# wonjune-kang/llm-speech-summarization

Hardware: AMD Instinct MI355X
Metric: generated tokens/s of end-to-end generate_audio_response steps (encode + prefill + 256-token greedy decode), HuBERT-large -> Llama-3.2-3B; audio-sec/s reported beside it, encoder stage alone and in the pipeline (higher is better)
Workload: dtype bf16

## Files before the change

### llm-speech-summarization_amd/csrc/api.hip

```cpp
#include <stdarg.h>
#include <stdlib.h>

#include <atomic>
#include <mutex>

#include "common.h"

static thread_local char g_err[512] = "";

void sl_set_error(const char* fmt, ...) {
  va_list ap;
  va_start(ap, fmt);
  vsnprintf(g_err, sizeof(g_err), fmt, ap);
  va_end(ap);
}

extern "C" const char* sl_last_error(void) { return g_err; }

extern "C" int sl_version(void) { return SL_ABI_VERSION; }

extern "C" int sl_kv_quantize_e4m3_host(const float* x, uint8_t* out, int64_t n) {
  SL_CHECK_ARG(x != nullptr && out != nullptr && n >= 0, "sl_kv_quantize_e4m3_host: bad arguments");
  for (int64_t i = 0; i < n; ++i) out[i] = (uint8_t)sl_q8_e4m3(x[i]);
  return 0;
}

extern "C" int sl_device_arch(char* buf, int n) {
  SL_CHECK_ARG(buf != nullptr && n > 0, "sl_device_arch: bad buffer");
  int dev = 0;
  SL_HIP(hipGetDevice(&dev));
  hipDeviceProp_t prop;
  SL_HIP(hipGetDeviceProperties(&prop, dev));
  snprintf(buf, (size_t)n, "%s", prop.gcnArchName);
  return 0;
}

static std::atomic<const SlEnv*> g_env{nullptr};
static std::mutex g_env_mu;

static int env_int(const char* name, int dflt) {
  const char* e = getenv(name);
  return (e && e[0]) ? atoi(e) : dflt;
}

static const SlEnv* env_load() {
  SlEnv& e = *new SlEnv();
  e.compact_pin = env_int("SL_COMPACT_PIN", 1);
  e.tape_fuse = env_int("SL_TAPE_FUSE", 1);
  e.attn_bwd_kf = env_int("SL_ATTN_BWD_KF", 0);
  e.decode_prefetch = env_int("SL_DECODE_PREFETCH", 0);
  e.attn_fwd_st = env_int("SL_ATTN_FWD_ST", 1);
  e.conv0_fold = env_int("SL_CONV0_FOLD", 1);
  e.enc_wt_ahead = env_int("SL_ENC_WT_AHEAD", 1);
  e.rms_bwd_lean = env_int("SL_RMSBWD_LEAN", 2);
  e.glds_ring = env_int("SL_GLDS_RING", 4);
  if (e.glds_ring != 3 && e.glds_ring != 4 && e.glds_ring != 104 && e.glds_ring != 204) e.glds_ring = 0;
  e.splitk_slots = env_int("SL_SPLITK_SLOTS", 0);
  e.glds_dmab = env_int("SL_GLDS_DMAB", 0);
  e.tt_ring = env_int("SL_TT_RING", 1);
  e.split_k256 = env_int("SL_SPLIT_K256", 1);
  e.ring_max_tiles = env_int("SL_GLDS_RING_MAX_TILES", 0);
  e.attn_bwd_both = env_int("SL_ATTN_BWD_BOTH", 1);
  e.wgrad_stream_min_tok = env_int("SL_WGRAD_STREAM_MIN_TOK", 0);
  e.tt_batched = env_int("SL_TT_BATCHED", 1);
  e.ln_colred_inkernel = env_int("SL_LN_COLRED_INKERNEL", 0);
  e.stream_min_m = env_int("SL_STREAM_MIN_M", 26);
  if (e.stream_min_m < 16) e.stream_min_m = 26;
  e.disable_t256 = getenv("SL_DISABLE_T256") != nullptr;
  e.t256_min_tiles = env_int("SL_T256_MIN_TILES", 512);
  e.t256_min_k = env_int("SL_T256_MIN_K", 1024);
  e.t256_phased = env_int("SL_T256_PHASED", 1);
  e.t256_by_rounds_pad = env_int("SL_T256_BY_ROUNDS_PAD", 1);
  e.decode_tiled = env_int("SL_DECODE_TILED", 1);
  e.stream_k = env_int("SL_STREAM_K", 1);
  e.split_k = env_int("SL_SPLIT_K", 1);
  e.wgrad_tr = env_int("SL_WGRAD_TR", 1);
  e.tt_max_splits = env_int("SL_TT_MAX_SPLITS", 8);
  e.lnbwd_nw = env_int("SL_LNBWD_NW", 16);
  e.skinny_alt = env_int("SL_SKINNY_ALT", 0);
  e.prefill_share_prefix = env_int("SL_PREFILL_SHARE_PREFIX", 1);
  e.prefill_prune_last = env_int("SL_PREFILL_PRUNE_LAST", 1);
  e.gemm_ko = env_int("SL_GEMM_KO", 0);
  { const char* sp = getenv("SL_GEMM_STAMP_PTR"); e.gemm_stamp_ptr = (sp && sp[0]) ? strtoull(sp, nullptr, 16) : 0ull; }
  const char* g = getenv("SL_DISABLE_GLDS");
  e.disable_glds = (g && g[0] == '1') ? 1 : ((g && g[0] == '2') ? 2 : 0);
  e.direct_epilogue = env_int("SL_DIRECT_EPILOGUE", 0);
  e.gemm_gm = env_int("SL_GEMM_GM", 8);
  e.attn_full_min = env_int("SL_ATTN_FULL_MIN", 32);
  e.attn_force_split = getenv("SL_ATTN_FORCE_SPLIT") != nullptr;
  { const int ks = env_int("SL_ATTN_DECODE_KS", 128); e.attn_decode_ks = (ks == 64 || ks == 65) ? ks : 128; }
  e.attn_split_merge = env_int("SL_ATTN_SPLIT_MERGE", -1);
  e.attn_generic = env_int("SL_ATTN_GENERIC", 0);
  e.attn_qt = env_int("SL_ATTN_QT", 0);
  e.norm_single_row = env_int("SL_NORM_SINGLE_ROW", 0);
  e.no_ln_fold = env_int("SL_NO_LN_FOLD", 0);
  e.no_swap_epilogue = env_int("SL_NO_SWAP_EPILOGUE", 0);
  e.gemm_log = env_int("SL_GEMM_LOG", 0);
  e.no_wgrad_stream = env_int("SL_NO_WGRAD_STREAM", 0);
  e.stream_splits = e.stream_nwv = e.stream_mt = 0;
  e.stream_nl = env_int("SL_STREAM_NL", 0);
  e.stream_wide = env_int("SL_STREAM_WIDE", 1);
  e.stream_wsplits = env_int("SL_STREAM_WSPLITS", 0);
  e.stream_fixup = env_int("SL_STREAM_FIXUP", 0);
  const char* sc = getenv("SL_STREAM_CFG");
  if (sc && sc[0]) {
    int sp = 0, nwv = 0, mt = 0;
    const int n = sscanf(sc, "%d,%d,%d", &sp, &nwv, &mt);
    if (n >= 2) {
      if (sp >= 1 && sp <= 64) e.stream_splits = sp;
      if (nwv == 2 || nwv == 4) e.stream_nwv = nwv;
    }
    if (n == 3 && (mt == 8 || mt == 16)) e.stream_mt = mt;
  }
  return &e;
}

const SlEnv& sl_env() {
  const SlEnv* e = g_env.load(std::memory_order_acquire);
  if (!e) {
    std::lock_guard<std::mutex> lk(g_env_mu);
    e = g_env.load(std::memory_order_relaxed);
    if (!e) {
      e = env_load();
      g_env.store(e, std::memory_order_release);
    }
  }
  return *e;
}

static thread_local int g_family_rows = 0;
int sl_family_rows(int rows) { return g_family_rows > rows ? g_family_rows : rows; }
int sl_family_pin(int rows) {
  const int prev = g_family_rows;
  g_family_rows = rows > 0 ? rows : 0;
  return prev;
}

extern "C" int sl_tuning_reload(void) {
  std::lock_guard<std::mutex> lk(g_env_mu);
  g_env.store(env_load(), std::memory_order_release);
  return 0;
}
```

### llm-speech-summarization_amd/csrc/common.h

```cpp
#pragma once
#include <hip/hip_runtime.h>
#include <stdint.h>
#include <stdio.h>
#include <string.h>

#include "../../include/speechllm.h"

void sl_set_error(const char* fmt, ...);

#define SL_CHECK_ARG(cond, ...)      \
  do {                               \
    if (!(cond)) {                   \
      sl_set_error(__VA_ARGS__);     \
      return SL_ERR_ARG;             \
    }                                \
  } while (0)

#define SL_CHECK_LAUNCH(what)                                                        \
  do {                                                                               \
    hipError_t e__ = hipGetLastError();                                              \
    if (e__ != hipSuccess) {                                                         \
      sl_set_error("%s: %s", what, hipGetErrorString(e__));                          \
      return SL_ERR_LAUNCH;                                                          \
    }                                                                                \
// ... 196 lines not shown
  }
};

__device__ __forceinline__ float gelu_erf(float x) { return 0.5f * x * (1.0f + erff(x * 0.70710678118654752440f)); }
__device__ __forceinline__ float gelu_fast(float x) {
  const float z = fabsf(x) * 0.70710678118654752440f;
  const float t = __builtin_amdgcn_rcpf(__builtin_fmaf(0.3275911f, z, 1.0f));
  float pl = __builtin_fmaf(0.5f * 1.061405429f, t, 0.5f * -1.453152027f);
  pl = __builtin_fmaf(pl, t, 0.5f * 1.421413741f);
  pl = __builtin_fmaf(pl, t, 0.5f * -0.284496736f);
  pl = __builtin_fmaf(pl, t, 0.5f * 0.254829592f);
  const float w = pl * t * __builtin_amdgcn_exp2f(-1.4426950408889634f * z * z);
  return __builtin_fmaf(-fabsf(x), w, fmaxf(x, 0.f));
}
__device__ __forceinline__ uint32_t lowbias32(uint32_t x) {
  x ^= x >> 16; x *= 0x7feb352du; x ^= x >> 15; x *= 0x846ca68bu; x ^= x >> 16;
  return x;
}
__device__ __forceinline__ bool dropout_keep(int64_t i, uint64_t seed, uint32_t thr24) {
  const uint32_t h = lowbias32((uint32_t)i ^ lowbias32((uint32_t)((uint64_t)i >> 32) ^ (uint32_t)seed) ^ (uint32_t)(seed >> 32));
  return (h >> 8) >= thr24;
}
__device__ __forceinline__ uint32_t drop_inner(uint32_t hi, uint64_t seed) { return lowbias32(hi ^ (uint32_t)seed) ^ (uint32_t)(seed >> 32); }
__device__ __forceinline__ bool dropout_keep_lo(uint32_t lo, uint32_t inner, uint32_t thr24) { return (lowbias32(lo ^ inner) >> 8) >= thr24; }
template <typename T> __device__ __forceinline__ float gelu_act(float x) {
  if constexpr (sizeof(T) == 2) return gelu_fast(x);
  else return gelu_erf(x);
}
__device__ __forceinline__ float silu(float x) { return x / (1.0f + __expf(-x)); }
__device__ __forceinline__ float gelu_grad(float u) {
  const float cdf = 0.5f * (1.0f + erff(u * 0.70710678118654752440f));
  const float pdf = 0.39894228040143267794f * __expf(-0.5f * u * u);
  return cdf + u * pdf;
}

__device__ __forceinline__ float wave_sum(float v) {
#pragma unroll
  for (int o = 32; o > 0; o >>= 1) v += __shfl_xor(v, o, 64);
  return v;
}
__device__ __forceinline__ float wave_max(float v) {
#pragma unroll
  for (int o = 32; o > 0; o >>= 1) v = fmaxf(v, __shfl_xor(v, o, 64));
  return v;
}

constexpr int SL_MAX_DEVICES = 64;

static inline int64_t ceil_div64(int64_t a, int64_t b) { return (a + b - 1) / b; }

#define SL_DISPATCH_DTYPE_INF(dtype, T, ...)                  \
  do {                                                        \
    if ((dtype) == SL_F32) {                                  \
      using T = float;                                        \
      __VA_ARGS__;                                            \
    } else if ((dtype) == SL_BF16) {                          \
      using T = bf16_t;                                       \
      __VA_ARGS__;                                            \
    } else if ((dtype) == SL_F16) {                           \
      using T = f16_t;                                        \
      __VA_ARGS__;                                            \
    } else {                                                  \
      sl_set_error("unknown dtype %d", (int)(dtype));         \
      return SL_ERR_ARG;                                      \
    }                                                         \
  } while (0)
#define SL_DISPATCH_DTYPE(dtype, T, ...)                      \
  do {                                                        \
    if ((dtype) == SL_F32) {                                  \
      using T = float;                                        \
      __VA_ARGS__;                                            \
    } else if ((dtype) == SL_BF16) {                          \
      using T = bf16_t;                                       \
      __VA_ARGS__;                                            \
    } else {                                                  \
      sl_set_error("unknown dtype %d", (int)(dtype));         \
      return SL_ERR_ARG;                                      \
    }                                                         \
  } while (0)

static inline size_t sl_dtype_size(int dtype) { return dtype == SL_F32 ? 4 : 2; }
static inline bool sl_is16(int dtype) { return dtype == SL_BF16 || dtype == SL_F16; }
static inline int sl_kv_format_check(const char* who, int kv_format, int dtype, int head_dim) {
  if (kv_format != SL_KV_MODEL_DTYPE && kv_format != SL_KV_FP8_E4M3) {
    sl_set_error("%s: unknown K/V cache format %d (0 = model dtype, 1 = fp8 e4m3)", who, kv_format);
    return SL_ERR_ARG;
  }
  if (kv_format == SL_KV_FP8_E4M3 && !sl_is16(dtype)) {
    sl_set_error("%s: the fp8 K/V cache is built for bf16 / fp16 models, not dtype %d (float32 is the parity mode)", who, dtype);
    return SL_ERR_UNSUPPORTED;
  }
  if (kv_format == SL_KV_FP8_E4M3 && head_dim != 128) {
    sl_set_error("%s: the fp8 K/V cache is built for head_dim 128, not %d", who, head_dim);
    return SL_ERR_UNSUPPORTED;
  }
  return 0;
}
static inline size_t sl_kv_elem_size(int kv_format, int dtype) { return kv_format == SL_KV_FP8_E4M3 ? 1 : sl_dtype_size(dtype); }

struct SlEnv {
  int attn_fwd_st;
  int conv0_fold;
  int enc_wt_ahead;
  int glds_ring;
  int tt_batched;
  int wgrad_stream_min_tok;
  int attn_bwd_both;
  int ring_max_tiles;
  int split_k256;
  int ln_colred_inkernel;
  int tt_ring;
  int glds_dmab;
  int splitk_slots;
  int rms_bwd_lean;
  int decode_prefetch;
  int attn_bwd_kf;
  int tape_fuse;
  int compact_pin;
  int stream_min_m;
  int disable_t256;
  int t256_min_tiles;
  int t256_min_k;
  int t256_by_rounds_pad;
  int t256_phased;
  int disable_glds;
  int direct_epilogue;
  int gemm_gm;
  int attn_full_min;
  int attn_force_split;
  int attn_decode_ks;
  int attn_split_merge;
  int attn_generic;
  int attn_qt;
  int norm_single_row;
  int no_ln_fold;
  int no_wgrad_stream;
  int gemm_log;
  int no_swap_epilogue;
  int decode_tiled;
  int prefill_share_prefix;
  int prefill_prune_last;
  int skinny_alt;
  int tt_max_splits;
  int lnbwd_nw;
  int wgrad_tr;
  int split_k;
  int stream_k;
  int gemm_ko;
  unsigned long long gemm_stamp_ptr;
  int stream_splits, stream_nwv, stream_mt;
  int stream_wide;
  int stream_wsplits;
  int stream_fixup;
  int stream_nl;
};
const SlEnv& sl_env();

#define SL_TRANSPOSE_BATCH 64
struct SlTransposeRec {
  const void* x; void* y;
  int64_t ldx, ldy;
  int32_t rows, cols, ld_out, tiles_r;
};
struct SlTransposeBatch {
  SlTransposeRec rec[SL_TRANSPOSE_BATCH];
  int32_t first_block[SL_TRANSPOSE_BATCH];
  int32_t n, pad;
};
int sl_transpose_pad_batch_impl(const SlTransposeRec* recs, int n, int32_t dtype, sl_stream stream);
int sl_family_rows(int rows);
int sl_family_pin(int rows);
struct SlFamilyPin {
  int prev;
  explicit SlFamilyPin(int rows) : prev(sl_family_pin(rows)) {}
  ~SlFamilyPin() { sl_family_pin(prev); }
};
```

### llm-speech-summarization_amd/csrc/gemm.hip

```cpp
#include <stdlib.h>

#include "common.h"
#include "gemm_internal.h"

#include "gemm_epilogue.h"

template <typename T, int ACT>
__global__ __launch_bounds__(256, 2) void gemm_tiled_kernel(GemmP p) {
  constexpr int VEC = Vec16<T>::VEC;
  constexpr int BK = TROWB / (int)sizeof(T);
  __shared__ __attribute__((aligned(16))) unsigned char smem[2][2][TBM * TROWB];

  const int tid = threadIdx.x, lane = tid & 63, wave = tid >> 6;
  const int wm = wave >> 1, wn = wave & 1;
  const int r = lane & 15, q = lane >> 4;

  int bm, bn;
  tile_patch_coords(xcd_remap(blockIdx.x, p.tiles_m * p.tiles_n), p.tiles_m, p.tiles_n, 8, bm, bn);
  const int z = blockIdx.y;

  int64_t a_off; int wz;
  if (!resolve_group(p, z, bm, a_off, wz)) return;
  const T* A = (const T*)p.A + a_off;
  const T* W = (const T*)p.W + (int64_t)wz * p.sW + p.wx;
// ... 788 lines not shown
        if (p.post == SL_POST_DROPOUT) post_ok = !p.colsum && !p.ln_mr && !p.stats_out && (act == SL_ACT_GELU ? (p.aux && !p.res) : (p.res && !p.aux));
        if (p.post == SL_POST_GELU_BWD || p.post == SL_POST_SILU_MUL_BWD)
          post_ok = act == SL_ACT_NONE && !(p.post_ld & 7) && !((uintptr_t)p.post_in & 15) && (p.post == SL_POST_GELU_BWD || !p.colsum);
        if (swap_store_ok(p, e, true) && form && !p.grp && !p.amax_val && post_ok && (phased || (!p.post && !p.colsum))) {
          pl.form = phased ? SL_T256_PHASED_SW : SL_T256_PLAIN_SW;
#ifdef SL_GEMM_DEBUG
          if (act == SL_ACT_NONE && phased && !p.ln_mr && (e.gemm_stamp_ptr || e.gemm_ko))
            pl.form = SL_T256_DBG + (e.gemm_stamp_ptr ? 8 : (e.gemm_ko >= 1 && e.gemm_ko <= 4 ? e.gemm_ko : 6));
#endif
        }
      }
      return pl;
    }
  }
  pl.tile(p, TBM);
  pl.grid = dim3(pl.tiles_m * pl.tiles_n, batch);
  const bool glds = whole_slabs(p, bk) && (!p.grp_ext || p.grp_kslab) && glds_on(e);
  if ((p.post || p.colsum) && !glds) { pl.fam = TP_UNSUPPORTED; return pl; }
  if (es == 2 && ring_ok(p, batch, bk, e, cus)) { pl.fam = TP_RING128; pl.form = e.glds_ring; }
  else if (whole_slabs(p, bk) && !p.grp_ext && e.disable_glds == 2) { pl.fam = TP_GLDS128; pl.form = GLDS_PLAIN; }
  else if (glds) { pl.fam = TP_GLDS128; pl.form = (es == 2 && e.glds_dmab && !p.grp_ext) ? GLDS_DMAB : GLDS_ASM; }
  else pl.fam = TP_REG128;
  return pl;
}

static void log_plan(const TiledPlan& pl) {
  static const char* const fam[] = {"reg128", "glds128", "ring128", "t256", "sk", "tt", "unsupported"};
  static const char* const glds[] = {"asm", "dmab", "plain"}, * const t256[] = {"phased", "phased_sw", "plain", "plain_sw", "sk", "sk_sw"};
  static const char* const tt[] = {"two_stage", "ring", "batched"}, * const close[] = {"none", "reduce", "defer"};
  char num[16];
  snprintf(num, sizeof(num), pl.fam == TP_T256 ? "dbg%d" : "%d", pl.form);
  const bool k256 = (pl.fam == TP_T256 || pl.fam == TP_SK) && pl.form < 6;
  const char* form = pl.fam == TP_GLDS128 ? glds[pl.form] : k256 ? t256[pl.form] : pl.fam == TP_TT ? tt[pl.form] : (pl.fam == TP_RING128 || pl.fam == TP_T256) ? num : "none";
  fprintf(stderr, "SLPLAN fam=%s form=%s tm=%d tn=%d grid=%u,%u,%u S=%d krun=%d close=%s\n", fam[pl.fam], form, pl.tiles_m, pl.tiles_n, pl.grid.x, pl.grid.y,
          pl.grid.z, pl.S, pl.krun, close[pl.close]);
}

template <typename T, int ACT>
static int run_tiled(const GemmP& p0, const TiledPlan& pl, void* sk_ws, const SlEnv& e, hipStream_t st) {
  if (pl.fam == TP_UNSUPPORTED) {
    sl_set_error("sl_gemm_ex: post_op / colsum_out need whole 128-byte K slabs (K %% %d == 0) and the LDS-DMA kernels (SL_DISABLE_GLDS unset)", TROWB / (int)sizeof(T));
    return SL_ERR_UNSUPPORTED;
  }
  float* part = (float*)((unsigned char*)sk_ws + SK_FLAG_BYTES);
  GemmP p = pl.runs ? partial_gemm(p0, pl.runs, pl.S, pl.krun, part) : p0;
  p.tiles_m = pl.tiles_m; p.tiles_n = pl.tiles_n;
#ifdef SL_GEMM_DEBUG
  if (pl.fam == TP_T256 && pl.form >= SL_T256_DBG) p.stamp = (uint32_t*)(uintptr_t)e.gemm_stamp_ptr;
#endif
  if (pl.fam == TP_TT) SL_TRY(sl_gemm_tt_kernel_launch(p, pl.form, pl.grid, pl.krun, st));
  else if (pl.fam == TP_T256 || pl.fam == TP_SK)
    SL_TRY((sl_gemm256_launch<T, ACT>(p, pl.form, pl.grid, pl.fam == TP_SK ? sk_ws : nullptr, st)));
  else if (pl.fam == TP_RING128) SL_TRY((sl_gemm128_ring_launch<T, ACT>(p, pl.form, pl.grid, st)));
  else {
    if (pl.fam == TP_REG128) hipLaunchKernelGGL((gemm_tiled_kernel<T, ACT>), pl.grid, dim3(256), 0, st, p);
    else if (pl.form == GLDS_PLAIN) hipLaunchKernelGGL((gemm_tiled_glds_kernel<T, ACT, false>), pl.grid, dim3(256), 0, st, p);
    else if (pl.form == GLDS_ASM) hipLaunchKernelGGL((gemm_tiled_glds_kernel<T, ACT, true>), pl.grid, dim3(256), 0, st, p);
    else if constexpr (sizeof(T) == 2) hipLaunchKernelGGL((gemm_tiled_glds_kernel<T, ACT, true, true>), pl.grid, dim3(256), 0, st, p);
    SL_CHECK_LAUNCH("gemm_tiled");
  }
  if (pl.close == CLOSE_DEFER) *p0.defer = pl.S;
  if (pl.close == CLOSE_REDUCE) {
    const int64_t vecs = ((int64_t)p0.M * p0.N + 3) / 4;
    hipLaunchKernelGGL((splitk_reduce_kernel<T>), dim3((unsigned)((vecs + 255) / 256)), dim3(256), 0, st, part, pl.S, (int64_t)p0.M * p0.N, p0);
    SL_CHECK_LAUNCH("splitk_reduce");
  }
  return 0;
}

template <typename T, int MT, int ACT, int RF, int NW, int U, bool PACKED, bool KCONT = false, bool W8 = false>
static int launch_skinny_cfg(GemmP& p, const SkinnyX& sx, int batch, hipStream_t st) {
  dim3 grid((p.N + 16 * RF - 1) / (16 * RF), batch);
  hipLaunchKernelGGL((gemm_skinny_kernel<T, MT, ACT, RF, NW, U, PACKED, KCONT, W8>), grid, dim3(NW * 64), 0, st, p, sx);
  SL_CHECK_LAUNCH("gemm_skinny");
  return 0;
}

template <typename T, int MT, int ACT, bool PACKED>
static int launch_skinny_mt(GemmP& p, const SkinnyX& sx, int batch, const SlEnv& e, hipStream_t st) {
  constexpr bool PAIRS = (ACT == SL_ACT_SILU_MUL || ACT == SL_ACT_ROPE_KV);
  const int nfrag = (p.N + 15) / 16 * batch;
  if constexpr (MT == 1) {
    if constexpr (PACKED && sizeof(T) == 2 && !PAIRS) {
      if (nfrag < 256 && sl_family_rows(p.M) <= 8 && !(e.skinny_alt & 1)) {
        const int per_wave = p.K / 32 / 16;
        if (per_wave % 3 == 0) return launch_skinny_cfg<T, MT, ACT, 1, 16, 3, PACKED>(p, sx, batch, st);
        return launch_skinny_cfg<T, MT, ACT, 1, 16, 4, PACKED>(p, sx, batch, st);
      }
    }
    if (nfrag >= 1024) return launch_skinny_cfg<T, MT, ACT, 4, 4, 4, PACKED>(p, sx, batch, st);
    if (nfrag >= 256 || PAIRS) return launch_skinny_cfg<T, MT, ACT, 2, 8, 4, PACKED>(p, sx, batch, st);
    if constexpr (!PAIRS) return launch_skinny_cfg<T, MT, ACT, 1, 16, 2, PACKED>(p, sx, batch, st);
  } else if constexpr (MT == 2) {
    if (nfrag >= 1024) return launch_skinny_cfg<T, MT, ACT, 2, 8, 4, PACKED>(p, sx, batch, st);
    if (nfrag >= 256 || PAIRS) return launch_skinny_cfg<T, MT, ACT, 2, 16, 2, PACKED>(p, sx, batch, st);
    if constexpr (!PAIRS) return launch_skinny_cfg<T, MT, ACT, 1, 16, 2, PACKED>(p, sx, batch, st);
  } else {
    if (nfrag >= 1024) return launch_skinny_cfg<T, MT, ACT, 4, 8, 2, PACKED>(p, sx, batch, st);
    if (nfrag >= 256 || PAIRS) return launch_skinny_cfg<T, MT, ACT, 2, 16, 2, PACKED>(p, sx, batch, st);
    if constexpr (!PAIRS) return launch_skinny_cfg<T, MT, ACT, 1, 16, 2, PACKED>(p, sx, batch, st);
  }
  return 0;
}

template <typename T, int MT, int ACT, int RF, int NW, int UA = 4>
static int launch_skinny_w8_u(GemmP& p, const SkinnyX& sx, hipStream_t st) {
  const int pw = p.K / 64 / NW;
  if (pw % UA != 0 && pw % 3 == 0) return launch_skinny_cfg<T, MT, ACT, RF, NW, 3, true, false, true>(p, sx, 1, st);
  return launch_skinny_cfg<T, MT, ACT, RF, NW, UA, true, false, true>(p, sx, 1, st);
}
template <typename T, int MT, int ACT>
static int launch_skinny_w8_mt(GemmP& p, const SkinnyX& sx, hipStream_t st) {
  constexpr bool PAIRS = (ACT == SL_ACT_SILU_MUL || ACT == SL_ACT_ROPE_KV);
  const int nfrag = (p.N + 15) / 16;
  if (nfrag >= 1024) return launch_skinny_w8_u<T, MT, ACT, MT == 1 ? 4 : 2, MT == 1 ? 4 : 8>(p, sx, st);
  if (nfrag >= 256 || PAIRS) return launch_skinny_w8_u<T, MT, ACT, 2, MT == 1 ? 8 : 16, MT == 1 ? 4 : 2>(p, sx, st);
  if constexpr (!PAIRS) return launch_skinny_w8_u<T, MT, ACT, 1, 16>(p, sx, st);
  return 0;
}
template <typename T>
static int launch_skinny_w8(GemmP& p, const SkinnyX& sx, int act, hipStream_t st) {
  const bool mt1 = sl_family_rows(p.M) <= 16;
  switch (act) {
    case SL_ACT_NONE: return mt1 ? launch_skinny_w8_mt<T, 1, SL_ACT_NONE>(p, sx, st) : launch_skinny_w8_mt<T, 2, SL_ACT_NONE>(p, sx, st);
    case SL_ACT_SILU_MUL: return mt1 ? launch_skinny_w8_mt<T, 1, SL_ACT_SILU_MUL>(p, sx, st) : launch_skinny_w8_mt<T, 2, SL_ACT_SILU_MUL>(p, sx, st);
    default: return mt1 ? launch_skinny_w8_mt<T, 1, SL_ACT_ROPE_KV>(p, sx, st) : launch_skinny_w8_mt<T, 2, SL_ACT_ROPE_KV>(p, sx, st);
  }
}

template <typename T, int ACT>
static int launch_skinny(GemmP& p, const SkinnyX& sx, int batch, bool packed, const SlEnv& e, hipStream_t st) {
  if (packed) {
    if constexpr (ACT == SL_ACT_GELU) {
      sl_set_error("sl_gemm: packed weights are not built with the GELU epilogue");
      return SL_ERR_UNSUPPORTED;
    } else {
      if (sl_family_rows(p.M) <= 16) return launch_skinny_mt<T, 1, ACT, true>(p, sx, batch, e, st);
      if (sl_family_rows(p.M) <= 32) return launch_skinny_mt<T, 2, ACT, true>(p, sx, batch, e, st);
      return launch_skinny_mt<T, 4, ACT, true>(p, sx, batch, e, st);
    }
  }
  if constexpr (ACT == SL_ACT_ROPE_KV) {
    sl_set_error("sl_gemm: the ROPE_KV epilogue needs packed weights");
    return SL_ERR_UNSUPPORTED;
  } else {
    if (sl_family_rows(p.M) <= 16) return launch_skinny_mt<T, 1, ACT, false>(p, sx, batch, e, st);
    if (sl_family_rows(p.M) <= 32) return launch_skinny_mt<T, 2, ACT, false>(p, sx, batch, e, st);
    return launch_skinny_mt<T, 4, ACT, false>(p, sx, batch, e, st);
  }
}

template <typename T>
static int gemm_typed(const sl_gemm_args* a, GemmP& p, const SkinnyX& sx, hipStream_t st, void* sk_ws, size_t sk_ws_bytes, const SlEnv& e) {
  const bool skinny = sl_family_rows(a->M) <= 64 && !p.ta && !p.tw && !p.res_f32 && !p.grp && no_rider(p) && !p.post && !p.colsum;
  const bool packed = a->w_layout == SL_W_PACKED;
  if (!skinny && (packed || a->act == SL_ACT_ROPE_KV || sx.fuse_rms)) {
    sl_set_error("sl_gemm: packed weights / ROPE_KV / fused RMSNorm need plain operands (no transposes / groups), M=%d", a->M);
    return SL_ERR_UNSUPPORTED;
  }
  SL_CHECK_ARG(a->act >= SL_ACT_NONE && a->act <= SL_ACT_ROPE_KV, "sl_gemm: unknown act %d", a->act);
  const bool dry = e.gemm_log == 2;
  if (!skinny) {
    const TiledPlan pl = plan_tiled(p, a->batch, a->dtype, a->act, sk_ws ? sk_ws_bytes : 0, e, dry ? 256 : sk_cu_count());
    if (e.gemm_log) log_plan(pl);
    if (dry && pl.fam != TP_UNSUPPORTED) return 0;
    if (a->act == SL_ACT_NONE) return run_tiled<T, SL_ACT_NONE>(p, pl, sk_ws, e, st);
    if (a->act == SL_ACT_GELU) return run_tiled<T, SL_ACT_GELU>(p, pl, sk_ws, e, st);
    return run_tiled<T, SL_ACT_SILU_MUL>(p, pl, sk_ws, e, st);
  }
  if (dry) return 0;
  switch (a->act) {
    case SL_ACT_NONE: return launch_skinny<T, SL_ACT_NONE>(p, sx, a->batch, packed, e, st);
    case SL_ACT_GELU: return launch_skinny<T, SL_ACT_GELU>(p, sx, a->batch, packed, e, st);
    case SL_ACT_SILU_MUL: return launch_skinny<T, SL_ACT_SILU_MUL>(p, sx, a->batch, packed, e, st);
    default: return launch_skinny<T, SL_ACT_ROPE_KV>(p, sx, a->batch, packed, e, st);
  }
}

int sl_gemm_impl(const sl_gemm_args* a, const sl_gemm_fused* fx, const sl_gemm_ex_args* ex, hipStream_t st) {
  SL_CHECK_ARG(a != nullptr, "sl_gemm: null args");
  const SlEnv& e = sl_env();
  SL_CHECK_ARG(a->M > 0 && a->N > 0 && a->K > 0 && a->batch > 0, "sl_gemm: bad shape M=%d N=%d K=%d batch=%d", a->M, a->N, a->K, a->batch);
  SL_CHECK_ARG(a->dtype == SL_F32 || sl_is16(a->dtype), "sl_gemm: bad dtype %d", a->dtype);
  const int vec = a->dtype == SL_F32 ? 4 : 8;
  const bool both_t = ex && ex->trans_a && ex->trans_w;
  SL_CHECK_ARG(both_t || a->K % vec == 0, "sl_gemm: K=%d must be a multiple of %d", a->K, vec);
  SL_CHECK_ARG(a->lda % vec == 0 && a->strideA % vec == 0, "sl_gemm: lda/strideA must keep rows 16-byte aligned");
  SL_CHECK_ARG(((uintptr_t)a->A & 15) == 0 && ((uintptr_t)a->W & 15) == 0, "sl_gemm: A and W must be 16-byte aligned");
  const bool w8 = a->w_layout == SL_W_PACKED_E4M3;
  if (w8) {
    if (a->dtype == SL_F32) {
      sl_set_error("sl_gemm: e4m3 weight images (w_layout %d) are built for bf16 / fp16, not float32 (the parity mode)", a->w_layout);
      return SL_ERR_UNSUPPORTED;
    }
    SL_CHECK_ARG(a->K % 64 == 0, "sl_gemm: e4m3 weight images need K %% 64 == 0 (K=%d)", a->K);
    SL_CHECK_ARG(a->batch == 1 && !ex && a->act != SL_ACT_GELU, "sl_gemm: e4m3 weight images take one plain product (batch 1, no sl_gemm_ex features, no GELU)");
    if (sl_family_rows(a->M) > sl_w8_max_rows()) {
      sl_set_error("sl_gemm: e4m3 weight images are built for the skinny kernels, up to sl_w8_max_rows() = %d rows (M=%d)", sl_w8_max_rows(), sl_family_rows(a->M));
      return SL_ERR_UNSUPPORTED;
    }
  } else if (a->w_layout == SL_W_PACKED) {
    SL_CHECK_ARG(a->K % (4 * vec) == 0, "sl_gemm: packed weights need K %% %d == 0", 4 * vec);
  } else {
    SL_CHECK_ARG(a->w_layout == SL_W_ROWMAJOR, "sl_gemm: unknown w_layout %d", a->w_layout);
    SL_CHECK_ARG(a->ldw % vec == 0 && a->strideW % vec == 0, "sl_gemm: ldw/strideW must keep rows 16-byte aligned");
  }
  if (a->act == SL_ACT_SILU_MUL) SL_CHECK_ARG(a->N % 32 == 0, "sl_gemm: SILU_MUL needs N %% 32 == 0 (16-row gate/up blocks)");
  GemmP p = {};
  p.A = a->A; p.lda = a->lda; p.sA = a->strideA;
  p.W = a->W; p.ldw = a->ldw; p.sW = a->strideW;
  p.C = a->C; p.ldc = a->ldc; p.sC = a->strideC;
  p.bias = a->bias; p.sBias = a->strideBias;
  p.res = a->residual; p.ldr = a->ldr; p.sR = a->strideR;
  p.M = a->M; p.N = a->N; p.K = a->K; p.out_f32 = a->out_f32;
  p.w_mod = 1; p.drop_scale = 1.f;
  p.direct_epi = e.direct_epilogue;
  p.gm = e.gemm_gm;
  if (ex) {
    SL_CHECK_ARG(a->dtype != SL_F16 || !(ex->trans_a || ex->trans_w || ex->post_op || ex->colsum_out || ex->aux_out),
                 "sl_gemm_ex: trans_a / trans_w / post_op / colsum_out / aux_out are training features, not built for SL_F16");
    p.ta = ex->trans_a; p.tw = ex->trans_w; p.aux = ex->aux_out; p.res_f32 = ex->residual_f32;
    p.grp = ex->groups; p.w_mod = ex->w_mod > 0 ? ex->w_mod : 1;
    if (ex->deferred_splits) { *ex->deferred_splits = 0; p.defer = ex->deferred_splits; }
    p.grp_ext = ex->groups && ex->groups_ext;
    p.grp_kslab = ex->groups && ex->groups_ext == 2;
    SL_CHECK_ARG(!(p.ta || p.tw || p.aux) || a->act != SL_ACT_SILU_MUL, "sl_gemm_ex: transposed operands / aux_out are not combined with SILU_MUL");
    SL_CHECK_ARG(!p.res_f32 || a->out_f32, "sl_gemm_ex: residual_f32 needs out_f32");
    SL_CHECK_ARG(!(p.ta || p.tw) || a->w_layout == SL_W_ROWMAJOR, "sl_gemm_ex: transposed operands need row-major storage");
    if (ex->ln_mr || ex->ln_u || ex->ln_c || ex->stats_out) {
      SL_CHECK_ARG(rows_epilogue_ok(e, a->M, a->N, a->K, a->dtype) && a->batch == 1 && !ex->groups && !ex->trans_a && !ex->trans_w && !ex->aux_out &&
                       a->act != SL_ACT_SILU_MUL && a->w_layout == SL_W_ROWMAJOR && a->ldc % 4 == 0 && ((uintptr_t)a->C & 7) == 0 &&
                       (!a->residual || (a->ldr % 4 == 0 && ((uintptr_t)a->residual & 7) == 0)),
                   "sl_gemm_ex: ln_* / stats_out need a plain bf16 row-major product the LDS-DMA tiled kernels take (M=%d N=%d K=%d), 4-element aligned rows", a->M, a->N, a->K);
      SL_CHECK_ARG((!ex->ln_mr && !ex->ln_u && !ex->ln_c) || (ex->ln_mr && ex->ln_u && ex->ln_c && !a->bias),
                   "sl_gemm_ex: the LayerNorm fold needs ln_mr, ln_u and ln_c together (the bias is inside ln_c)");
      p.ln_mr = ex->ln_mr; p.ln_u = ex->ln_u; p.ln_c = ex->ln_c; p.stats_out = ex->stats_out;
    }
    if (ex->colsum_out && ex->trans_a && ex->trans_w && !ex->post_op) {
      p.colsum = ex->colsum_out;
      SL_CHECK_ARG(tt_ok(p, a->batch, a->dtype, e) && a->act == SL_ACT_NONE,
                   "sl_gemm_ex: colsum_out with trans_a + trans_w needs the token-major weight-gradient kernel (bf16, M and N multiples of 128, K >= 128, 8-element aligned rows; sl_gemm_tt_ok)");
    } else if (ex->post_op || ex->colsum_out) {
      SL_CHECK_ARG(ex->post_op >= SL_POST_NONE && ex->post_op <= SL_POST_SILU_MUL_BWD, "sl_gemm_ex: unknown post_op %d", ex->post_op);
      SL_CHECK_ARG(!ex->trans_a && !ex->trans_w && !ex->groups && !ex->ln_mr && !ex->ln_u && !ex->ln_c && !ex->stats_out && !ex->amax_val && !ex->amax_idx &&
                       a->batch == 1 && a->w_layout == SL_W_ROWMAJOR && a->act != SL_ACT_SILU_MUL && a->act != SL_ACT_ROPE_KV && a->M > 64,
                   "sl_gemm_ex: post_op / colsum_out need one plain row-major product on the tiled kernels (M > 64, no transposes / groups / ln_* / stats_out / amax_*)");
      SL_CHECK_ARG(ex->drop_p >= 0.f && ex->drop_p < 1.f, "sl_gemm_ex: drop_p %f outside [0, 1)", (double)ex->drop_p);
      if (ex->post_op == SL_POST_DROPOUT) SL_CHECK_ARG(ex->drop_p > 0.f && ex->drop_ld >= a->N, "sl_gemm_ex: SL_POST_DROPOUT needs drop_p > 0 and drop_ld >= N");
      if (ex->post_op == SL_POST_GELU_BWD)
        SL_CHECK_ARG(ex->post_in && ex->post_ld >= a->N && !a->residual && !a->bias && a->act == SL_ACT_NONE && !ex->aux_out && !a->out_f32 && (ex->drop_p == 0.f || ex->drop_ld >= a->N),
                     "sl_gemm_ex: SL_POST_GELU_BWD needs post_in (M, N), the plain epilogue (no bias / residual / act / aux_out) and an output in the storage type");
      if (ex->post_op == SL_POST_SILU_MUL_BWD)
        SL_CHECK_ARG(ex->post_in && ex->post_ld >= 2 * (int64_t)a->N && a->ldc >= 2 * (int64_t)a->N && a->N % 16 == 0 && !a->residual && !a->bias && a->act == SL_ACT_NONE &&
                         !ex->aux_out && !a->out_f32 && !ex->colsum_out && ex->drop_p == 0.f,
                     "sl_gemm_ex: SL_POST_SILU_MUL_BWD needs post_in = gu (M, 2 N), ldc >= 2 N, N %% 16 == 0 and the plain epilogue");
      p.post = ex->post_op; p.post_in = ex->post_in; p.post_ld = ex->post_ld; p.colsum = ex->colsum_out;
      if (ex->drop_p > 0.f && ex->post_op != SL_POST_NONE) {
        p.drop_thr24 = (uint32_t)((double)ex->drop_p * 16777216.0);
        p.drop_scale = 1.0f / (1.0f - ex->drop_p);
        p.drop_seed = ex->drop_seed; p.drop_ld = ex->drop_ld;
      }
    }
    if (ex->amax_val || ex->amax_idx) {
      SL_CHECK_ARG(ex->amax_val && ex->amax_idx && a->act == SL_ACT_NONE && a->batch == 1 && !ex->groups && !ex->trans_a && !ex->trans_w && !ex->aux_out &&
                       !a->residual && sl_family_rows(a->M) > 64 && a->w_layout == SL_W_ROWMAJOR,
                   "sl_gemm_ex: amax_val / amax_idx (fused row-wise top-1) need both pointers, the plain epilogue without residual, one "
                   "un-grouped row-major product and M > 64 (M=%d act=%d batch=%d)", a->M, a->act, a->batch);
      p.amax_val = ex->amax_val; p.amax_idx = ex->amax_idx;
    }
  }
  SL_CHECK_ARG(p.amax_val || a->C, "sl_gemm: null C");
  if (e.gemm_log)
    fprintf(stderr, "SLGEMM M=%d N=%d K=%d batch=%d act=%d ta=%d tw=%d res=%d resf32=%d outf32=%d aux=%d grp=%d bias=%d packed=%d dt=%d\n", a->M, a->N, a->K, a->batch, a->act,
            p.ta, p.tw, a->residual != nullptr, p.res_f32, a->out_f32, p.aux != nullptr, p.grp ? (p.grp_ext ? 2 : 1) : 0, a->bias != nullptr, a->w_layout == SL_W_PACKED, a->dtype);
  SkinnyX sx;
  memset(&sx, 0, sizeof(sx));
  if (fx) {
    sx.fuse_rms = fx->fuse_rms; sx.eps = fx->rms_eps;
    sx.cos = fx->rope_cos; sx.sin = fx->rope_sin; sx.pos = fx->tok_pos; sx.seq = fx->tok_seq;
    sx.kc = fx->k_cache; sx.vc = fx->v_cache; sx.nh = fx->n_heads; sx.nkv = fx->n_kv_heads; sx.max_ctx = fx->max_ctx;
    sx.rstd_in = fx->rstd_in; sx.rstd_out = fx->rstd_out; sx.norm_out = fx->norm_out; sx.norm_gain = fx->norm_gain;
    SL_CHECK_ARG((!fx->norm_out && !fx->norm_gain) || (fx->norm_out && fx->norm_gain && fx->rstd_out && !a->out_f32), "sl_gemm: norm_out needs norm_gain, rstd_out and an output in the storage type");
  }
  if (a->act == SL_ACT_ROPE_KV) {
    SL_CHECK_ARG(fx && fx->rope_cos && fx->rope_sin && fx->tok_pos && fx->tok_seq && fx->k_cache && fx->v_cache,
                 "sl_gemm: ROPE_KV epilogue needs the sl_gemm_fused tables");
    SL_CHECK_ARG(a->N == (fx->n_heads + 2 * fx->n_kv_heads) * 128 && a->batch == 1, "sl_gemm: ROPE_KV expects N = (n_heads + 2 n_kv) * 128");
    SL_TRY(sl_kv_format_check("sl_gemm (ROPE_KV)", fx->reserved, a->dtype, 128));
    sx.kv8 = fx->reserved == SL_KV_FP8_E4M3;
  }
  if (a->w_layout == SL_W_PACKED && sl_family_rows(a->M) > e.stream_min_m && a->batch == 1 && !ex && a->act != SL_ACT_GELU &&
      a->K % slab_elems(a->dtype) == 0)
    return e.gemm_log == 2 ? 0 : sl_gemm_stream_launch(p, sx, a->dtype, a->act, fx ? fx->split_ws : nullptr, fx ? fx->split_ws_bytes : 0, st);
  SL_CHECK_ARG(a->w_layout != SL_W_PACKED || sl_family_rows(a->M) <= 64, "sl_gemm: packed weights with M=%d > 64 need batch 1 and K %% 64 == 0", a->M);
  if (w8) {
    SL_CHECK_ARG(a->act >= SL_ACT_NONE && a->act <= SL_ACT_ROPE_KV, "sl_gemm: unknown act %d", a->act);
    SL_CHECK_ARG(!sx.rstd_out && !sx.norm_out && (!sx.rstd_in || sx.fuse_rms), "sl_gemm: e4m3 weight images take rstd_in (with fuse_rms) but not rstd_out / norm_out");
    if (e.gemm_log == 2) return 0;
    return a->dtype == SL_F16 ? launch_skinny_w8<f16_t>(p, sx, a->act, st) : launch_skinny_w8<bf16_t>(p, sx, a->act, st);
  }
  SL_CHECK_ARG(!sx.rstd_in && !sx.rstd_out && !sx.norm_out, "sl_gemm: rstd_in / rstd_out / norm_out are features of the streaming path (M > %d rows, packed weights)", e.stream_min_m);
  void* sk_ws = ex ? ex->sk_ws : nullptr;
  const size_t sk_ws_bytes = ex ? ex->sk_ws_bytes : 0;
  SL_CHECK_ARG(!sk_ws || ((uintptr_t)sk_ws & 15) == 0, "sl_gemm_ex: sk_ws must be 16-byte aligned");
  if (a->dtype == SL_F32) return gemm_typed<float>(a, p, sx, st, sk_ws, sk_ws_bytes, e);
  if (a->dtype == SL_F16) return gemm_typed<f16_t>(a, p, sx, st, sk_ws, sk_ws_bytes, e);
  return gemm_typed<bf16_t>(a, p, sx, st, sk_ws, sk_ws_bytes, e);
}

extern "C" int32_t sl_gemm_split_count(int32_t M, int32_t N, int32_t K, int32_t dtype) {
  M = sl_family_rows(M);
  if (M <= sl_env().stream_min_m || M <= 0 || N <= 0 || K <= 0 || K % (dtype == SL_F32 ? 32 : 64) != 0) return 1;
  return sl_gemm_stream_splits(M, N, K, dtype);
}

extern "C" size_t sl_gemm_split_workspace_bytes(int32_t M, int32_t N, int32_t K, int32_t dtype) {
  if (sl_family_rows(M) <= sl_env().stream_min_m || M <= 0 || N <= 0 || K <= 0) return 0;
  return sl_gemm_stream_ws_bytes(M, N, K, dtype);
}

extern "C" int32_t sl_gemm_ln_fold_ok(int32_t M, int32_t N, int32_t K, int32_t dtype) { return sl_gemm_rows_epilogue_ok(M, N, K, dtype) ? 1 : 0; }

extern "C" int sl_gemm(const sl_gemm_args* a, sl_stream stream) { return sl_gemm_impl(a, nullptr, nullptr, (hipStream_t)stream); }

extern "C" int sl_gemm_ex(const sl_gemm_args* a, const sl_gemm_ex_args* ex, sl_stream stream) {
  SL_CHECK_ARG(ex != nullptr, "sl_gemm_ex: null ex args");
  return sl_gemm_impl(a, nullptr, ex, (hipStream_t)stream);
}

extern "C" int sl_gemm_fused_decode(const sl_gemm_args* a, const sl_gemm_fused* fx, sl_stream stream) {
  SL_CHECK_ARG(fx != nullptr, "sl_gemm_fused_decode: null fused args");
  return sl_gemm_impl(a, fx, nullptr, (hipStream_t)stream);
}
```

### llm-speech-summarization_amd/csrc/gemm_epilogue.h

```cpp
#pragma once
#include "common.h"
#include "gemm_internal.h"

template <typename T, int MT, int NT>
__device__ __forceinline__ void tile_argmax(const GemmP& p, f32x4 (&acc)[MT][NT], int row_base, int col_base, int q, int r, int wz) {
  static_assert(NT == 4, "one 64-column group per wave");
  if (col_base >= p.N) return;
  const T* bias = p.bias ? (const T*)p.bias + (int64_t)wz * p.sBias : nullptr;
  const int64_t g = col_base >> 6;
#pragma unroll
  for (int m = 0; m < MT; ++m) {
    float bv[4];
    int bi[4];
#pragma unroll
    for (int i = 0; i < 4; ++i) { bv[i] = -INFINITY; bi[i] = 0x7fffffff; }
#pragma unroll
    for (int n = 0; n < NT; ++n) {
      const int col = col_base + n * 16 + r;
      if (col >= p.N) continue;
      const float b = bias ? to_f32(bias[col]) : 0.f;
#pragma unroll
      for (int i = 0; i < 4; ++i) {
        const float v = acc[m][n][i] + b;
        if (v > bv[i] || (v == bv[i] && col < bi[i])) { bv[i] = v; bi[i] = col; }
      }
    }
#pragma unroll
    for (int o = 1; o < 16; o <<= 1) {
#pragma unroll
      for (int i = 0; i < 4; ++i) {
        const float ov = __shfl_xor(bv[i], o, 64);
        const int oi = __shfl_xor(bi[i], o, 64);
        if (ov > bv[i] || (ov == bv[i] && oi < bi[i])) { bv[i] = ov; bi[i] = oi; }
      }
    }
    if (r == 0) {
#pragma unroll
      for (int i = 0; i < 4; ++i) {
        const int row = row_base + m * 16 + 4 * q + i;
        if (row < p.M) { p.amax_val[g * p.M + row] = bv[i]; p.amax_idx[g * p.M + row] = bi[i]; }
      }
    }
  }
}

template <typename T, int ACT, int MT, int NT>
__device__ __forceinline__ void tile_epilogue_g(const GemmP& p, f32x4 (&acc)[MT][NT], int row_base, int col_base, int q, int r, int z, int wz) {
  if constexpr (ACT == SL_ACT_NONE && NT == 4) {
    if (p.amax_val) { tile_argmax<T, MT, NT>(p, acc, row_base, col_base, q, r, wz); return; }
  }
  const int64_t co = (int64_t)z * p.sC + p.cx, ro = (int64_t)z * p.sR + p.rx;
  void* Cb = p.out_f32 ? (void*)((float*)p.C + co) : (void*)((T*)p.C + co);
  const T* bias = p.bias ? (const T*)p.bias + (int64_t)wz * p.sBias : nullptr;
  const void* Rb = p.res ? (p.res_f32 ? (const void*)((const float*)p.res + ro) : (const void*)((const T*)p.res + ro)) : nullptr;
  const int row0 = row_base + q * 4;
  const int col0 = col_base + r;
  if constexpr (ACT == SL_ACT_SILU_MUL) {
    static_assert(NT % 2 == 0, "gate/up fragments come in pairs");
    const int nout = p.N >> 1;
#pragma unroll
    for (int pr = 0; pr < NT / 2; ++pr) {
      const int gcol = col0 + (2 * pr) * 16, ucol = gcol + 16;
      const int ocol = (col_base >> 1) + pr * 16 + r;
      if (ocol >= nout) continue;
      const float bg = bias ? to_f32(bias[gcol]) : 0.f, bu = bias ? to_f32(bias[ucol]) : 0.f;
#pragma unroll
      for (int m = 0; m < MT; ++m)
#pragma unroll
        for (int i = 0; i < 4; ++i) {
          const int row = row0 + m * 16 + i;
          if (row < p.M) store_out<T>(p, Cb, Rb, row, ocol, silu(acc[m][2 * pr][i] + bg) * (acc[m][2 * pr + 1][i] + bu));
        }
    }
  } else {
#pragma unroll
    for (int n = 0; n < NT; ++n) {
      const int col = col0 + n * 16;
      if (col >= p.N) continue;
      const float b = bias ? to_f32(bias[col]) : 0.f;
      float csum = 0.f;
      constexpr int MG = ACT == SL_ACT_GELU ? 1 : (MT < 4 ? MT : 4);
#pragma unroll
      for (int mg = 0; mg < MT; mg += MG) {
        float rv[MG][4];
        if (Rb) {
#pragma unroll
          for (int m = 0; m < MG; ++m)
#pragma unroll
            for (int i = 0; i < 4; ++i) {
              int row = row0 + (mg + m) * 16 + i;
              row = row < p.M ? row : p.M - 1;
              rv[m][i] = p.res_f32 ? ((const float*)Rb)[(int64_t)row * p.ldr + col] : to_f32(((const T*)Rb)[(int64_t)row * p.ldr + col]);
            }
        }
#pragma unroll
        for (int m = 0; m < MG; ++m)
#pragma unroll
          for (int i = 0; i < 4; ++i) {
            const int row = row0 + (mg + m) * 16 + i;
            if (row < p.M) {
              float v = acc[mg + m][n][i] + b;
              if (p.aux) ((T*)p.aux + co)[(int64_t)row * p.ldc + col] = from_f32<T>(v);
              if constexpr (ACT == SL_ACT_GELU) v = gelu_act<T>(v);
              if (p.post == SL_POST_SILU_MUL_BWD) {
                const int64_t o = (int64_t)row * p.post_ld + 32 * (col >> 4) + (col & 15);
                float dg, du;
                post_silu_bwd<T>(v, to_f32(((const T*)p.post_in)[o]), to_f32(((const T*)p.post_in)[o + 16]), dg, du);
                T* op = (T*)Cb + (int64_t)row * p.ldc + 32 * (col >> 4) + (col & 15);
                op[0] = from_f32<T>(dg); op[16] = from_f32<T>(du);
                continue;
              }
              if (p.post) { float v1[1] = {v}; post_apply<T, 1>(p, row, col, v1); v = v1[0]; }
              if (Rb) v += rv[m][i];
              store_out<T>(p, Cb, nullptr, row, col, v);
              if (p.colsum) csum += p.out_f32 ? v : round_as<T>(v);
            }
          }
      }
      if (p.colsum) {
        csum += __shfl_xor(csum, 16, 64);
        csum += __shfl_xor(csum, 32, 64);
        if (q == 0) atomicAdd(p.colsum + col, csum);
      }
    }
  }
}

__device__ __forceinline__ void ld4(const float* ptr, float (&f)[4]) {
  const f32x4 v = *(const f32x4*)ptr;
  f[0] = v[0]; f[1] = v[1]; f[2] = v[2]; f[3] = v[3];
}
__device__ __forceinline__ void ld4(const bf16_t* ptr, float (&f)[4]) {
  const uint2 u = *(const uint2*)ptr;
  f[0] = bf16_bits_to_f32(u.x & 0xffffu); f[1] = bf16_bits_to_f32(u.x >> 16);
  f[2] = bf16_bits_to_f32(u.y & 0xffffu); f[3] = bf16_bits_to_f32(u.y >> 16);
}
__device__ __forceinline__ void ld4(const f16_t* ptr, float (&f)[4]) {
  const uint2 u = *(const uint2*)ptr;
  const f32x2_t a = unpack2<f16_t>(u.x), b = unpack2<f16_t>(u.y);
  f[0] = a[0]; f[1] = a[1]; f[2] = b[0]; f[3] = b[1];
}
__device__ __forceinline__ void unpack4(const f32x4& v, float (&f)[4]) { f[0] = v[0]; f[1] = v[1]; f[2] = v[2]; f[3] = v[3]; }
template <typename T> __device__ __forceinline__ void unpack4_16(const uint2& u, float (&f)[4]);
template <> __device__ __forceinline__ void unpack4_16<bf16_t>(const uint2& u, float (&f)[4]) {
  f[0] = bf16_bits_to_f32(u.x & 0xffffu); f[1] = bf16_bits_to_f32(u.x >> 16);
  f[2] = bf16_bits_to_f32(u.y & 0xffffu); f[3] = bf16_bits_to_f32(u.y >> 16);
}
template <> __device__ __forceinline__ void unpack4_16<f16_t>(const uint2& u, float (&f)[4]) {
  const f32x2_t a = unpack2<f16_t>(u.x), b = unpack2<f16_t>(u.y);
  f[0] = a[0]; f[1] = a[1]; f[2] = b[0]; f[3] = b[1];
}
template <typename T> __device__ __forceinline__ void unpack4r(const f32x4& v, float (&f)[4]) { unpack4(v, f); }
template <typename T> __device__ __forceinline__ void unpack4r(const uint2& u, float (&f)[4]) { unpack4_16<T>(u, f); }
__device__ __forceinline__ void st4(float* ptr, const float (&f)[4]) { *(f32x4*)ptr = f32x4{f[0], f[1], f[2], f[3]}; }
__device__ __forceinline__ void st4(bf16_t* ptr, const float (&f)[4]) { *(uint2*)ptr = make_uint2(pack2_bf16(f[0], f[1]), pack2_bf16(f[2], f[3])); }
__device__ __forceinline__ void st4(f16_t* ptr, const float (&f)[4]) { *(uint2*)ptr = make_uint2(pack2_f16(f[0], f[1]), pack2_f16(f[2], f[3])); }

__device__ __forceinline__ float row16_sum(float v) {
  v += __builtin_bit_cast(float, __builtin_amdgcn_update_dpp(0, __builtin_bit_cast(int, v), 0x128, 0xf, 0xf, false));
  v += __builtin_bit_cast(float, __builtin_amdgcn_update_dpp(0, __builtin_bit_cast(int, v), 0x124, 0xf, 0xf, false));
  v += __builtin_bit_cast(float, __builtin_amdgcn_update_dpp(0, __builtin_bit_cast(int, v), 0x122, 0xf, 0xf, false));
  v += __builtin_bit_cast(float, __builtin_amdgcn_update_dpp(0, __builtin_bit_cast(int, v), 0x121, 0xf, 0xf, false));
  return v;
}

enum : int { EPI_GENERIC = 1, EPI_RES = 2, EPI_LN = 4, EPI_STATS = 8, EPI_AUX = 16, EPI_POST = 32, EPI_SBWD = 64, EPI_DROP = 128, EPI_GBWD = 256 };

template <typename T, int ACT, int MT, int F>
__device__ __forceinline__ void tile_epilogue_rows_impl(const GemmP& p, f32x4 (&acc)[MT][4], int row_base, int col_base, int lane, int wz, float* wsm,
                                                        const float2* mr_lds, int64_t co, int64_t ro) {
  constexpr bool G = (F & EPI_GENERIC) != 0, BF = sizeof(T) == 2;
  const bool f_aux = G && p.aux != nullptr, f_out32 = G && p.out_f32, f_res32 = G && p.res && p.res_f32;
  const bool f_rest = G ? (p.res && !p.res_f32) : (F & EPI_RES) != 0;
  const bool f_ln = BF && (G ? p.ln_mr != nullptr : (F & EPI_LN) != 0);
  const bool f_stats = BF && (G ? p.stats_out != nullptr : (F & EPI_STATS) != 0);
  constexpr bool PO = (F & EPI_POST) != 0, SB = (F & EPI_SBWD) != 0;
  const int f_post = PO ? p.post : 0;
  const bool f_cs = PO && p.colsum != nullptr;
  const bool f_pin = PO && !SB && p.post == SL_POST_GELU_BWD;
  float cs[4] = {0.f, 0.f, 0.f, 0.f};
  const int q = lane >> 4, r = lane & 15;
  const int c4 = r * 4;
  const int col = col_base + c4;
  const bool col_ok = col < p.N;
  const int colc = col_ok ? col : 0;
  float b4[4] = {0.f, 0.f, 0.f, 0.f};
  if (p.bias && col_ok) {
    const T* bias = (const T*)p.bias + (int64_t)wz * p.sBias + col;
#pragma unroll
    for (int j = 0; j < 4; ++j) b4[j] = to_f32(bias[j]);
  }
  float u4[4] = {0.f, 0.f, 0.f, 0.f};
  if (f_ln && col_ok) {
#pragma unroll
    for (int j = 0; j < 4; ++j) { u4[j] = p.ln_u[col + j]; b4[j] = p.ln_c[col + j]; }
  }
  const int segs = (p.N + 63) >> 6, seg = col_base >> 6;
  using RawT = typename std::conditional<sizeof(T) == 2, uint2, f32x4>::type;
#pragma unroll
  for (int mg = 0; mg < MT; mg += 4) {
    RawT raw[16];
    RawT raw2[SB ? 16 : 1];
    if (f_rest) {
#pragma unroll
      for (int t = 0; t < 16; ++t) {
        int64_t row = row_base + mg * 16 + t * 4 + q;
        row = row < p.M ? row : p.M - 1;
        raw[t] = *(const RawT*)((const T*)p.res + ro + row * p.ldr + colc);
      }
    } else if (f_pin) {
#pragma unroll
      for (int t = 0; t < 16; ++t) {
        int64_t row = row_base + mg * 16 + t * 4 + q;
        row = row < p.M ? row : p.M - 1;
        raw[t] = *(const RawT*)((const T*)p.post_in + row * p.post_ld + colc);
      }
    }
    if constexpr (SB) {
#pragma unroll
      for (int t = 0; t < 16; ++t) {
        int64_t row = row_base + mg * 16 + t * 4 + q;
        row = row < p.M ? row : p.M - 1;
        const T* gp = (const T*)p.post_in + row * p.post_ld + 32 * (colc >> 4) + (colc & 15);
        raw[t] = *(const RawT*)gp;
// ... 382 lines not shown
```

### llm-speech-summarization_amd/csrc/gemm_internal.h

```cpp
#pragma once
#include "common.h"

struct GemmP {
  const void* A; int64_t lda, sA;
  const void* W; int64_t ldw, sW;
  void* C; int64_t ldc, sC;
  const void* bias; int64_t sBias;
  const void* res; int64_t ldr, sR;
  int M, N, K, out_f32;
  int tiles_m, tiles_n;
  int ta, tw;
  void* aux;
  int res_f32;
  const int64_t* grp;
  int w_mod;
  int64_t cx, rx, wx;
  int grp_ext;
  int grp_kslab;
  int gm;
  int direct_epi;
  const float* ln_mr;
  const float* ln_u;
  const float* ln_c;
  float* stats_out;
  float* amax_val;
  int* amax_idx;
  int post;
  uint32_t drop_thr24;
  float drop_scale;
  uint64_t drop_seed;
  int64_t drop_ld;
  const void* post_in; int64_t post_ld;
  float* colsum;
  int32_t* defer;
  int krun;
  uint32_t* stamp;
};

__device__ __forceinline__ bool resolve_group(GemmP& p, int z, int bm, int64_t& a_off, int& wz, int tile_rows = 128) {
  p.cx = 0; p.rx = 0; p.wx = 0;
  wz = z;
  a_off = (int64_t)z * p.sA;
  if (p.grp) {
    const int64_t* g = p.grp + (p.grp_ext ? 8 : 4) * (int64_t)z;
    p.M = (int)g[0];
    if (p.grp_ext) { p.wx = g[4]; p.N = (int)g[5]; p.K = (int)g[6]; }
    a_off = g[1];
    p.cx = g[2] - (int64_t)z * p.sC;
    p.rx = g[3] - (int64_t)z * p.sR;
    wz = z % p.w_mod;
    if (bm * tile_rows >= p.M) return false;
  }
  return true;
}

__device__ __forceinline__ int xcd_remap(int bid, int n) {
  const int qn = n >> 3, rn = n & 7, xcd = bid & 7, idx = bid >> 3;
  return (xcd < rn ? xcd * (qn + 1) : rn * (qn + 1) + (xcd - rn) * qn) + idx;
}
__device__ __forceinline__ void tile_patch_coords(int v, int tiles_m, int tiles_n, int gm, int& bm, int& bn) {
  const int per = gm * tiles_n, grp = v / per, first = grp * gm;
  const int gsz = (tiles_m - first) < gm ? (tiles_m - first) : gm;
  const int in = v - grp * per;
  bm = first + in % gsz;
  bn = in / gsz;
}

template <typename T>
__device__ __forceinline__ void store_out(const GemmP& p, void* Cb, const void* Rb, int64_t row, int64_t col, float v) {
  if (Rb) v += p.res_f32 ? ((const float*)Rb)[row * p.ldr + col] : to_f32(((const T*)Rb)[row * p.ldr + col]);
  if (p.out_f32)
    ((float*)Cb)[row * p.ldc + col] = v;
  else
    ((T*)Cb)[row * p.ldc + col] = from_f32<T>(v);
}

template <typename T> __device__ __forceinline__ float round_as(float v) { return to_f32(from_f32<T>(v)); }
template <> __device__ __forceinline__ float round_as<float>(float v) { return v; }

template <typename T, int NV>
__device__ __forceinline__ void post_drop(const GemmP& p, int64_t row, int col, float (&v)[NV]) {
  if (!p.drop_thr24) return;
  const int64_t i0 = row * p.drop_ld + col;
  const uint32_t inner = drop_inner((uint32_t)((uint64_t)i0 >> 32), p.drop_seed);
  const uint32_t inner2 = drop_inner((uint32_t)((uint64_t)(i0 + NV - 1) >> 32), p.drop_seed);
#pragma unroll
  for (int j = 0; j < NV; ++j) {
    const int64_t i = i0 + j;
    const uint32_t in_ = ((uint64_t)i >> 32) == ((uint64_t)i0 >> 32) ? inner : inner2;
    v[j] = dropout_keep_lo((uint32_t)i, in_, p.drop_thr24) ? round_as<T>(v[j]) * p.drop_scale : 0.f;
  }
}

template <typename T, int NV>
__device__ __forceinline__ void post_apply(const GemmP& p, int64_t row, int col, float (&v)[NV]) {
  if (p.post == SL_POST_DROPOUT) {
    post_drop<T, NV>(p, row, col, v);
  } else if (p.post == SL_POST_GELU_BWD) {
    if (p.drop_thr24) {
      post_drop<T, NV>(p, row, col, v);
    }
    const T* pre = (const T*)p.post_in + row * p.post_ld + col;
#pragma unroll
    for (int j = 0; j < NV; ++j) v[j] = round_as<T>(v[j]) * gelu_grad(to_f32(pre[j]));
  }
}

template <typename T>
__device__ __forceinline__ void post_silu_bwd(float d, float g, float u, float& dg, float& du) {
  d = round_as<T>(d);
  const float sg = 1.0f / (1.0f + __expf(-g));
  dg = d * u * sg * (1.0f + g * (1.0f - sg));
  du = d * g * sg;
}

constexpr int TBM = 128, TBN = 128, TROWB = 128;

__device__ __forceinline__ int lds_off(int row, int ch) { return row * TROWB + ((ch ^ (row & 7)) << 4); }

typedef __attribute__((address_space(3))) void* lds_ptr_t;
typedef const __attribute__((address_space(1))) void* glb_ptr_t;

constexpr int XBM = 256, XBN = 256;
constexpr size_t SK_FLAG_BYTES = 1024, SK_SLOT_BYTES = (size_t)XBM * XBN * 4;
constexpr int SK_WS_SLOTS = 512;

enum : int { SL_T256_PHASED = 0, SL_T256_PHASED_SW = 1, SL_T256_PLAIN = 2, SL_T256_PLAIN_SW = 3, SL_T256_SK = 4, SL_T256_SK_SW = 5, SL_T256_DBG = 16 };
template <typename T, int ACT>
int sl_gemm256_launch(const GemmP& p, int kind, dim3 grid, void* sk_ws, hipStream_t st);
template <typename T, int ACT>
int sl_gemm128_ring_launch(const GemmP& p, int stages, dim3 grid, hipStream_t st);
enum : int { SL_TT_TWO_STAGE = 0, SL_TT_RING = 1, SL_TT_BATCHED = 2 };
int sl_gemm_tt_kernel_launch(const GemmP& p, int form, dim3 grid, int slabs_per_run, hipStream_t st);

bool sl_gemm_post_ok(int64_t M, int N, int K, int dtype);
bool sl_gemm_rows_epilogue_ok(int M, int N, int K, int dtype);

struct SkinnyX {
  const float* cos; const float* sin;
  const int32_t* pos; const int32_t* seq;
  void* kc; void* vc;
  int nh, nkv, max_ctx, fuse_rms;
  float eps;
  int kv8;
  const float* rstd_in;
  float* rstd_out;
  void* norm_out;
  const void* norm_gain;
};
constexpr int SL_ACT_ROPE_KV8 = 64 + SL_ACT_ROPE_KV;
constexpr bool sl_act_is_rope_kv(int act) { return act == SL_ACT_ROPE_KV || act == SL_ACT_ROPE_KV8; }
template <typename T>
__device__ __forceinline__ void kv_store(void* cache, int64_t at, float v, int kv8) {
  const T t = from_f32<T>(v);
  if constexpr (sizeof(T) == 2) {
    if (kv8) { ((uint8_t*)cache)[at] = (uint8_t)sl_q8_e4m3(to_f32(t)); return; }
  }
  ((T*)cache)[at] = t;
}

int sl_gemm_stream_launch(GemmP& p, const SkinnyX& sx, int dtype, int act, void* split_ws, size_t split_ws_bytes, hipStream_t st);
size_t sl_gemm_stream_ws_bytes(int M, int N, int K, int dtype);
int sl_gemm_stream_splits(int M, int N, int K, int dtype);
```

### llm-speech-summarization_amd/csrc/gemm_stream.hip

```cpp
#include <type_traits>
#include <stdlib.h>

#include <atomic>

#include "gemm_internal.h"

struct StreamX {
  float* part;
  float* part_ss;
  int splits, sps;
  int np;
  int* cnt;
  float* ss_part;
};

__device__ __forceinline__ void st_sc1_16(float* ptr, const f32x4& v) {
  asm volatile("global_store_dwordx4 %0, %1, off sc1" ::"v"(ptr), "v"(v) : "memory");
}
__device__ __forceinline__ void ld_sc1_16(f32x4& v, const float* ptr) {
  asm volatile("global_load_dwordx4 %0, %1, off sc1" : "=v"(v) : "v"(ptr) : "memory");
}
__device__ __forceinline__ void vm_drain16(f32x4 (&v)[16]) {
  asm volatile("s_waitcnt vmcnt(0)"
               : "+v"(v[0]), "+v"(v[1]), "+v"(v[2]), "+v"(v[3]), "+v"(v[4]), "+v"(v[5]), "+v"(v[6]), "+v"(v[7]), "+v"(v[8]), "+v"(v[9]), "+v"(v[10]),
// ... 372 lines not shown
    };
    dma(0);
    dma(1);
    asm volatile("s_waitcnt vmcnt(%0)" ::"n"(NDMA) : "memory");
    __builtin_amdgcn_s_barrier();
    for (int it = 0; it < n_it; ++it) {
      dma(it + 2);
      asm volatile("s_waitcnt vmcnt(%0)" ::"n"(NDMA) : "memory");
      __builtin_amdgcn_s_barrier();
    }
    asm volatile("s_waitcnt vmcnt(0)" ::: "memory");
  } else {
    uint4 fx[2][MTW], fw[2][RFW];
    auto rd = [&](int it, int s2, int set) {
      const unsigned char* sl_ = smem + (it % NSLOT) * SLOT;
#pragma unroll
      for (int t = 0; t < MTW; ++t) fx[set][t] = *(const uint4*)(sl_ + lds_off(wm * 64 + t * 16 + r, s2 * 4 + q));
#pragma unroll
      for (int f = 0; f < RFW; ++f) fw[set][f] = *(const uint4*)(sl_ + SLAB_X + ((wn * RFW + f) * 2 + s2) * 1024 + lane * 16);
    };
    auto mma = [&](int set) {
#pragma unroll
      for (int t = 0; t < MTW; ++t)
#pragma unroll
        for (int f = 0; f < RFW; ++f) MMA<T>::step(acc[f][t], fw[set][f], fx[set][t]);
      if constexpr (sizeof(T) == 2) {
#pragma unroll
        for (int i = 0; i < MTW + RFW; ++i) {
          __builtin_amdgcn_sched_group_barrier(0x008, 2, 0);
          __builtin_amdgcn_sched_group_barrier(0x100, 1, 0);
        }
      }
    };
    __builtin_amdgcn_s_barrier();
    rd(0, 0, 0);
    for (int it = 0; it < n_it; ++it) {
      __builtin_amdgcn_sched_barrier(0);
      rd(it, 1, 1);
      mma(0);
      __builtin_amdgcn_sched_barrier(0);
      asm volatile("s_waitcnt lgkmcnt(0)" ::: "memory");
      __builtin_amdgcn_s_barrier();
      rd(it + 1, 0, 0);
      mma(1);
      __builtin_amdgcn_sched_barrier(0);
    }
    stream_finish<T, MTW, ACT, RFW>(p, sx, s, acc, ssum, false, mw, sp, fi0, nfrag, false, q, r);
  }
  if (!(s.splits > 1 && s.cnt)) return;

  const bool cw = wave < CW;
  const int tile = nb * mblocks + mblock;
  asm volatile("s_waitcnt vmcnt(0)" ::: "memory");
  __builtin_amdgcn_s_barrier();
  if (tid == 0) {
    const int old = atomicAdd(&s.cnt[tile], 1);
    fx_last[0] = old == s.splits - 1;
    if (old == s.splits - 1) s.cnt[tile] = 0;
  }
  __builtin_amdgcn_s_barrier();
  if (!fx_last[0]) return;
  bool rowstat = false;
  if constexpr (ACT == SL_ACT_NONE) rowstat = sx.rstd_out != nullptr;
  if (cw) {
#pragma unroll
    for (int t = 0; t < MTW; ++t)
#pragma unroll
      for (int f = 0; f < RFW; ++f) acc[f][t] = f32x4{0.f, 0.f, 0.f, 0.f};
    for (int sp2 = 0; sp2 < s.splits; ++sp2) {
      f32x4 v[MTW * RFW];
#pragma unroll
      for (int t = 0; t < MTW; ++t) {
        int m = mw + t * 16 + r; m = m < p.M ? m : p.M - 1;
#pragma unroll
        for (int f = 0; f < RFW; ++f) {
          const int fi = fi0 + f < nfrag ? fi0 + f : nfrag - 1;
          ld_sc1_16(v[t * RFW + f], s.part + ((int64_t)sp2 * p.M + m) * s.np + fi * 16 + 4 * q);
        }
      }
      vm_drain16(v);
#pragma unroll
      for (int t = 0; t < MTW; ++t)
#pragma unroll
        for (int f = 0; f < RFW; ++f) acc[f][t] += v[t * RFW + f];
    }
    if (!rowstat) {
      StreamX s1 = s;
      s1.splits = 1;
      stream_finish<T, MTW, ACT, RFW>(p, sx, s1, acc, ssum, false, mw, sp, fi0, nfrag, false, q, r);
    }
  }
  if (!rowstat) return;
  if constexpr (ACT == SL_ACT_NONE) {
    if (cw) {
      const T* bias = (const T*)p.bias;
#pragma unroll
      for (int t = 0; t < MTW; ++t) {
        const int m = mw + t * 16 + r;
        float sq = 0.f;
        if (m < p.M) {
#pragma unroll
          for (int f = 0; f < RFW; ++f) {
#pragma unroll
            for (int i = 0; i < 4; ++i) {
              const int col = (fi0 + f) * 16 + 4 * q + i;
              if (col >= p.N) continue;
              float v = acc[f][t][i];
              if (bias) v += to_f32(bias[col]);
              if (p.res) v += p.res_f32 ? ((const float*)p.res)[(int64_t)m * p.ldr + col] : to_f32(((const T*)p.res)[(int64_t)m * p.ldr + col]);
              if (p.out_f32) {
                ((float*)p.C)[(int64_t)m * p.ldc + col] = v;
              } else {
                const T o = from_f32<T>(v);
                ((T*)p.C)[(int64_t)m * p.ldc + col] = o;
                v = to_f32(o);
              }
              sq = fmaf(v, v, sq);
            }
          }
        }
        sq += __shfl_xor(sq, 16);
        sq += __shfl_xor(sq, 32);
        if (q == 0) fx_ss[wm][wn][t * 16 + r] = sq;
      }
    }
    const int nbv = (nfrag + BF - 1) / BF;
    __builtin_amdgcn_s_barrier();
    if (tid < 256) {
      const int m = m0 + tid;
      if (m < p.M)
        __hip_atomic_store(&s.ss_part[(int64_t)nb * p.M + m], fx_ss[tid >> 6][0][tid & 63] + fx_ss[tid >> 6][1][tid & 63], __ATOMIC_RELAXED,
                           __HIP_MEMORY_SCOPE_AGENT);
    }
    asm volatile("s_waitcnt vmcnt(0)" ::: "memory");
    __builtin_amdgcn_s_barrier();
    if (tid == 0) {
      const int old = atomicAdd(&s.cnt[1024 + mblock], 1);
      fx_last[1] = old == nbv - 1;
      if (old == nbv - 1) s.cnt[1024 + mblock] = 0;
    }
    __builtin_amdgcn_s_barrier();
    if (!fx_last[1]) return;
    if (tid < 256) {
      const int m = m0 + tid;
      if (m < p.M) {
        float t = 0.f;
        for (int j = 0; j < nbv; ++j) t += __hip_atomic_load(&s.ss_part[(int64_t)j * p.M + m], __ATOMIC_RELAXED, __HIP_MEMORY_SCOPE_AGENT);
        sx.rstd_out[m] = rsqrtf(t / (float)p.N + sx.eps);
      }
    }
  }
}

template <int UN, int NCH, bool PAIRS>
__device__ __forceinline__ void reduce_add_splits(const float* rec, int64_t split_stride, int sp0, const uint32_t (&voff)[NCH], f32x4 (&a4)[NCH],
                                                  f32x4 (&b4)[NCH]) {
  f32x4 va[NCH][UN], vb[NCH][UN];
#pragma unroll
  for (int u = 0; u < UN; ++u) {
    const float* row = rec + (int64_t)(sp0 + u) * split_stride;
#pragma unroll
    for (int j = 0; j < NCH; ++j) {
      va[j][u] = *(const f32x4*)(row + voff[j]);
      if constexpr (PAIRS) vb[j][u] = *(const f32x4*)(row + voff[j] + 16);
    }
  }
#pragma unroll
  for (int u = 0; u < UN; ++u)
#pragma unroll
    for (int j = 0; j < NCH; ++j) {
      a4[j] += va[j][u];
      if constexpr (PAIRS) b4[j] += vb[j][u];
    }
}
template <int UNMAX, int NCH, bool PAIRS>
__device__ __forceinline__ void reduce_sum_splits(const float* rec, int64_t split_stride, int splits, const uint32_t (&voff)[NCH], f32x4 (&a4)[NCH],
                                                  f32x4 (&b4)[NCH]) {
  int sp0 = 0;
  for (; sp0 + UNMAX <= splits; sp0 += UNMAX) reduce_add_splits<UNMAX, NCH, PAIRS>(rec, split_stride, sp0, voff, a4, b4);
  if constexpr (UNMAX > 4) {
    if (splits - sp0 >= 4) { reduce_add_splits<4, NCH, PAIRS>(rec, split_stride, sp0, voff, a4, b4); sp0 += 4; }
  }
  if constexpr (UNMAX > 2) {
    if (splits - sp0 >= 2) { reduce_add_splits<2, NCH, PAIRS>(rec, split_stride, sp0, voff, a4, b4); sp0 += 2; }
  }
  if constexpr (UNMAX > 1) {
    if (splits - sp0 >= 1) reduce_add_splits<1, NCH, PAIRS>(rec, split_stride, sp0, voff, a4, b4);
  }
}

template <typename T, int ACT>
__global__ __launch_bounds__(256) void gemm_stream_reduce_kernel(GemmP p, SkinnyX sx, StreamX s) {
  constexpr bool PAIRS = (ACT == SL_ACT_SILU_MUL || sl_act_is_rope_kv(ACT));
  const int nfrag = (p.N + 15) >> 4;
  const int nunits = PAIRS ? (nfrag + 1) / 2 : nfrag;
  const int64_t idx = (int64_t)blockIdx.x * 256 + threadIdx.x;
  const int q = (int)(idx & 3);
  const int unit = (int)((idx >> 2) % nunits);
  const int m = (int)(idx / (4 * (int64_t)nunits));
  if (m >= p.M) return;
  const int gf = PAIRS ? 2 * unit : unit;
  f32x4 a4[1] = {{0.f, 0.f, 0.f, 0.f}}, b4[1] = {{0.f, 0.f, 0.f, 0.f}};
  const uint32_t voff[1] = {0u};
  reduce_sum_splits<8, 1, PAIRS>(s.part + (int64_t)m * s.np + gf * 16 + 4 * q, (int64_t)p.M * s.np, s.splits, voff, a4, b4);
  float ssum = 0.f;
  const bool stats_here = sx.fuse_rms && !sx.rstd_in;
  if (stats_here)
    for (int sp = 0; sp < s.splits; ++sp) ssum += s.part_ss[(int64_t)sp * p.M + m];
  const float rs = sx.rstd_in ? sx.rstd_in[m] : (stats_here ? rsqrtf(ssum / (float)p.K + sx.eps) : 1.0f);
  float a[4], b[4];
#pragma unroll
  for (int i = 0; i < 4; ++i) { a[i] = a4[0][i] * rs; b[i] = b4[0][i] * rs; }
  stream_epilogue4<T, ACT>(p, sx, m, gf, 4 * q, a, b);
}

template <typename T>
__device__ __forceinline__ float norm_round(float x, float rstd) {
  float y = x * rstd;
  asm volatile("" : "+v"(y));
  return to_f32(from_f32<T>(y));
}

template <typename T, int NCH, bool FAST>
__global__ __launch_bounds__(256) void gemm_stream_reduce_rowstat_kernel(GemmP p, SkinnyX sx, StreamX s) {
  __shared__ float wsum[16];
  const int nfrag = (p.N + 15) >> 4;
  const int ngroups = (4 * nfrag + 63) >> 6;
  const int m = blockIdx.x, tid = threadIdx.x;
  uint32_t col0[NCH], voff[NCH];
  bool live[NCH];
#pragma unroll
  for (int j = 0; j < NCH; ++j) {
    col0[j] = 4u * (uint32_t)(j * 256 + tid);
    live[j] = col0[j] < (FAST ? (uint32_t)p.N : 16u * (uint32_t)nfrag);
    voff[j] = live[j] ? col0[j] : 0u;
  }
  float kept[NCH][4];
  if constexpr (FAST) {
    typedef typename std::conditional<sizeof(T) == 2, uint2, f32x4>::type Piece;
    Piece rr[NCH];
#pragma unroll
    for (int j = 0; j < NCH; ++j) rr[j] = *(const Piece*)((const T*)p.res + (int64_t)m * p.ldr + voff[j]);
    f32x4 a4[NCH], b4[NCH];
#pragma unroll
    for (int j = 0; j < NCH; ++j) a4[j] = b4[j] = f32x4{0.f, 0.f, 0.f, 0.f};
    reduce_sum_splits<(NCH >= 3 ? 2 : 4), NCH, false>(s.part + (int64_t)m * s.np, (int64_t)p.M * s.np, s.splits, voff, a4, b4);
#pragma unroll
    for (int j = 0; j < NCH; ++j) {
      float v[4];
      if constexpr (sizeof(T) == 2) {
        const f32x2_t lo = unpack2<T>(rr[j].x), hi = unpack2<T>(rr[j].y);
        v[0] = a4[j][0] + lo.x; v[1] = a4[j][1] + lo.y; v[2] = a4[j][2] + hi.x; v[3] = a4[j][3] + hi.y;
        const uint32_t plo = pack2<T>(v[0], v[1]), phi = pack2<T>(v[2], v[3]);
        if (live[j]) *(uint2*)((T*)p.C + (int64_t)m * p.ldc + col0[j]) = make_uint2(plo, phi);
        const f32x2_t f01 = unpack2<T>(plo), f23 = unpack2<T>(phi);
        v[0] = f01.x; v[1] = f01.y; v[2] = f23.x; v[3] = f23.y;
      } else {
#pragma unroll
        for (int i = 0; i < 4; ++i) v[i] = a4[j][i] + rr[j][i];
        if (live[j]) *(f32x4*)((float*)p.C + (int64_t)m * p.ldc + col0[j]) = f32x4{v[0], v[1], v[2], v[3]};
      }
      float sq = 0.f;
#pragma unroll
      for (int i = 0; i < 4; ++i) { kept[j][i] = v[i]; sq = fmaf(v[i], v[i], sq); }
      sq = wave_sum(live[j] ? sq : 0.f);
      if ((tid & 63) == 0) wsum[j * 4 + (tid >> 6)] = sq;
    }
  } else {
  const bool res16 = !p.res_f32 && sizeof(T) == 2;
  const bool vec_res = p.res && !(p.ldr & 3) && !((uintptr_t)p.res & (res16 ? 7 : 15));
  const bool vec_c = !(p.ldc & 3) && !((uintptr_t)p.C & ((p.out_f32 || sizeof(T) == 4) ? 15 : 7));
  float r[NCH][4];
#pragma unroll
  for (int j = 0; j < NCH; ++j) {
#pragma unroll
    for (int i = 0; i < 4; ++i) r[j][i] = 0.f;
    if (!p.res || !live[j]) continue;
    const int64_t off = (int64_t)m * p.ldr + col0[j];
    if (vec_res && col0[j] + 3 < (uint32_t)p.N) {
      if (res16) {
        if constexpr (sizeof(T) == 2) {
          const uint2 w = *(const uint2*)((const T*)p.res + off);
          const f32x2_t lo = unpack2<T>(w.x), hi = unpack2<T>(w.y);
          r[j][0] = lo.x; r[j][1] = lo.y; r[j][2] = hi.x; r[j][3] = hi.y;
        }
      } else {
        const f32x4 w = *(const f32x4*)((const float*)p.res + off);
#pragma unroll
        for (int i = 0; i < 4; ++i) r[j][i] = w[i];
      }
    } else {
      for (int i = 0; i < 4 && col0[j] + i < (uint32_t)p.N; ++i)
        r[j][i] = p.res_f32 ? ((const float*)p.res)[off + i] : to_f32(((const T*)p.res)[off + i]);
    }
  }
  f32x4 a4[NCH], b4[NCH];
#pragma unroll
  for (int j = 0; j < NCH; ++j) a4[j] = b4[j] = f32x4{0.f, 0.f, 0.f, 0.f};
  reduce_sum_splits<(NCH >= 3 ? 2 : 4), NCH, false>(s.part + (int64_t)m * s.np, (int64_t)p.M * s.np, s.splits, voff, a4, b4);
  float ssum = 0.f;
  const bool stats_here = sx.fuse_rms && !sx.rstd_in;
  if (stats_here)
    for (int sp = 0; sp < s.splits; ++sp) ssum += s.part_ss[(int64_t)sp * p.M + m];
  const float rs = sx.rstd_in ? sx.rstd_in[m] : (stats_here ? rsqrtf(ssum / (float)p.K + sx.eps) : 1.0f);
  const T* bias = (const T*)p.bias;
#pragma unroll
  for (int j = 0; j < NCH; ++j) {
    float sq = 0.f;
#pragma unroll
    for (int i = 0; i < 4; ++i) kept[j][i] = 0.f;
    if (live[j]) {
      const int64_t off = (int64_t)m * p.ldc + col0[j];
      const bool whole = col0[j] + 3 < (uint32_t)p.N;
      float v[4];
#pragma unroll
      for (int i = 0; i < 4; ++i) {
        v[i] = a4[j][i] * rs;
        if (bias && col0[j] + i < (uint32_t)p.N) v[i] += to_f32(bias[col0[j] + i]);
        if (p.res) v[i] += r[j][i];
      }
      if (whole && vec_c) {
        if (p.out_f32) {
          *(f32x4*)((float*)p.C + off) = f32x4{v[0], v[1], v[2], v[3]};
        } else if constexpr (sizeof(T) == 2) {
          const uint32_t lo = pack2<T>(v[0], v[1]), hi = pack2<T>(v[2], v[3]);
          *(uint2*)((T*)p.C + off) = make_uint2(lo, hi);
          const f32x2_t f01 = unpack2<T>(lo), f23 = unpack2<T>(hi);
          v[0] = f01.x; v[1] = f01.y; v[2] = f23.x; v[3] = f23.y;
        } else {
          *(f32x4*)((float*)p.C + off) = f32x4{v[0], v[1], v[2], v[3]};
        }
#pragma unroll
        for (int i = 0; i < 4; ++i) { kept[j][i] = v[i]; sq = fmaf(v[i], v[i], sq); }
      } else {
#pragma unroll
        for (int i = 0; i < 4; ++i) {
          if (col0[j] + i >= (uint32_t)p.N) continue;
          if (p.out_f32) {
            ((float*)p.C)[off + i] = v[i];
          } else {
            const T o = from_f32<T>(v[i]);
            ((T*)p.C)[off + i] = o;
            v[i] = to_f32(o);
          }
          kept[j][i] = v[i];
          sq = fmaf(v[i], v[i], sq);
        }
      }
    }
    sq = wave_sum(sq);
    if ((tid & 63) == 0) wsum[j * 4 + (tid >> 6)] = sq;
  }
  }
  typedef typename std::conditional<sizeof(T) == 2, uint2, f32x4>::type GainPiece;
  GainPiece gg[NCH];
  if constexpr (FAST) {
    if (sx.norm_out) {
#pragma unroll
      for (int j = 0; j < NCH; ++j) gg[j] = *(const GainPiece*)((const T*)sx.norm_gain + voff[j]);
    }
  }
  __syncthreads();
  float t = 0.f;
  for (int g = 0; g < ngroups; ++g) t += wsum[g];
  const float rstd = rsqrtf(t / (float)p.N + sx.eps);
  if (tid == 0) sx.rstd_out[m] = rstd;
  if (sx.norm_out) {
    const bool vec_g = FAST || !((uintptr_t)sx.norm_gain & (sizeof(T) == 2 ? 7 : 15));
    const bool vec_n = FAST || (!(p.N & 3) && !((uintptr_t)sx.norm_out & (sizeof(T) == 2 ? 7 : 15)));
#pragma unroll
    for (int j = 0; j < NCH; ++j) {
      if (!live[j]) continue;
      const T* gain = (const T*)sx.norm_gain + col0[j];
      T* dst = (T*)sx.norm_out + (int64_t)m * p.N + col0[j];
      if (FAST || (col0[j] + 3 < (uint32_t)p.N && vec_n)) {
        float g4[4], o[4];
        if constexpr (FAST) {
          if constexpr (sizeof(T) == 2) {
            const f32x2_t lo = unpack2<T>(gg[j].x), hi = unpack2<T>(gg[j].y);
            g4[0] = lo.x; g4[1] = lo.y; g4[2] = hi.x; g4[3] = hi.y;
          } else {
#pragma unroll
            for (int i = 0; i < 4; ++i) g4[i] = gg[j][i];
          }
        } else if constexpr (sizeof(T) == 2) {
          if (vec_g) {
            const uint2 w = *(const uint2*)gain;
            const f32x2_t lo = unpack2<T>(w.x), hi = unpack2<T>(w.y);
            g4[0] = lo.x; g4[1] = lo.y; g4[2] = hi.x; g4[3] = hi.y;
          } else {
#pragma unroll
            for (int i = 0; i < 4; ++i) g4[i] = to_f32(gain[i]);
          }
        } else {
#pragma unroll
          for (int i = 0; i < 4; ++i) g4[i] = to_f32(gain[i]);
        }
#pragma unroll
        for (int i = 0; i < 4; ++i) o[i] = g4[i] * norm_round<T>(kept[j][i], rstd);
        if constexpr (sizeof(T) == 2) *(uint2*)dst = make_uint2(pack2<T>(o[0], o[1]), pack2<T>(o[2], o[3]));
        else *(f32x4*)dst = f32x4{o[0], o[1], o[2], o[3]};
      } else {
        for (int i = 0; i < 4 && col0[j] + i < (uint32_t)p.N; ++i)
          dst[i] = from_f32<T>(to_f32(gain[i]) * norm_round<T>(kept[j][i], rstd));
      }
    }
  }
}

struct StreamCfg { int mt, splits, nwv, d, nl; int wide, wsplits; };

static StreamCfg stream_cfg(int M, int N, int K, int kstep, bool have_ws, int dtype) {
  StreamCfg c;
  c.mt = M <= 32 ? 2 : (M <= 64 ? 4 : 8);
  const int nfrag = (N + 15) / 16;
  const int nst = K / (2 * kstep);
  c.d = 4;
  c.nl = sl_env().stream_nl ? sl_env().stream_nl : 1;
  const int sp_env = sl_env().stream_splits, nwv_env = sl_env().stream_nwv;
  if (sl_env().stream_mt && M > 64) c.mt = sl_env().stream_mt;
  const int mblocks = (M + c.mt * 16 - 1) / (c.mt * 16);
  c.nwv = ((nfrag + 7) / 8 * mblocks >= 512 || M > 128) && c.mt <= 8 ? 4 : 2;
  if (nwv_env && c.mt <= 8) c.nwv = nwv_env;
  const int base = mblocks * ((nfrag + c.nwv * 2 - 1) / (c.nwv * 2));
  int splits = 1;
  if (have_ws) {
    splits = 208 / base;
    const int max_splits = nst / 4 > 0 ? nst / 4 : 1;
    if (splits > max_splits) splits = max_splits;
    if (splits > 16) splits = 16;
    if (splits < 1) splits = 1;
  }
  if (sp_env && (have_ws || sp_env == 1)) splits = sp_env < nst ? sp_env : nst;
  c.splits = splits;
  c.wide = 0; c.wsplits = 1;
  if (sl_is16(dtype) && M > 384 && sl_env().stream_wide != 0) {
    const int wbase = ((M + 255) / 256) * ((nfrag + 7) / 8);
    if (wbase >= 128 || sl_env().stream_wide == 2) {
      c.wide = 1;
    }
    if (wbase < 128 && have_ws) {
      int ws_ = 240 / wbase;
      const int max_ws = nst / 6 > 0 ? nst / 6 : 1;
      if (ws_ > max_ws) ws_ = max_ws;
      if (ws_ > 8) ws_ = 8;
      if (sl_env().stream_wsplits) ws_ = sl_env().stream_wsplits < nst ? sl_env().stream_wsplits : nst;
      if (ws_ > 1) { c.wide = 1; c.wsplits = ws_; }
    }
  }
  return c;
}

static size_t stream_ws_header(int M) { return 8192 + (((size_t)32 * M * sizeof(float) + 255) & ~(size_t)255); }

int sl_gemm_stream_splits(int M, int N, int K, int dtype) {
  const StreamCfg c = stream_cfg(sl_family_rows(M), N, K, dtype == SL_F32 ? 16 : 32, true, dtype);
  return c.wide ? c.wsplits : c.splits;
}

size_t sl_gemm_stream_ws_bytes(int M, int N, int K, int dtype) {
  const size_t np = (size_t)((N + 15) / 16) * 16;
  const StreamCfg c = stream_cfg(sl_family_rows(M), N, K, dtype == SL_F32 ? 16 : 32, true, dtype);
  const int most = c.wide && c.wsplits > c.splits ? c.wsplits : c.splits;
  size_t splits = most > 1 ? (size_t)most : 0;
  return stream_ws_header(M) + splits * ((size_t)M * np + (size_t)M) * sizeof(float) + 256;
}

template <typename T, int ACT>
static int launch_stream_reduce(GemmP& p, const SkinnyX& sx, const StreamX& s, hipStream_t st) {
  if (s.splits <= 1) return 0;
  constexpr bool PAIRS = (ACT == SL_ACT_SILU_MUL || sl_act_is_rope_kv(ACT));
  const int nfrag = (p.N + 15) / 16;
  const int64_t nunits = PAIRS ? (nfrag + 1) / 2 : nfrag;
  const int64_t threads = (int64_t)p.M * nunits * 4;
  if constexpr (ACT == SL_ACT_NONE) {
    if (sx.rstd_out) {
      const uintptr_t al = sizeof(T) == 2 ? 7 : 15;
      const bool fast = !p.bias && p.res && !p.res_f32 && !p.out_f32 && !sx.fuse_rms && !sx.rstd_in && !(p.N & 3) && !(p.ldc & 3) && !(p.ldr & 3) &&
                        !((uintptr_t)p.C & al) && !((uintptr_t)p.res & al) && (!sx.norm_out || (!((uintptr_t)sx.norm_out & al) && !((uintptr_t)sx.norm_gain & al)));
      const int nch = (nfrag * 4 + 255) / 256;
#define SL_ROWSTAT_LAUNCH(NCH_)                                                                                                              \
  if (fast) hipLaunchKernelGGL((gemm_stream_reduce_rowstat_kernel<T, NCH_, true>), dim3(p.M), dim3(256), 0, st, p, sx, s);                   \
  else hipLaunchKernelGGL((gemm_stream_reduce_rowstat_kernel<T, NCH_, false>), dim3(p.M), dim3(256), 0, st, p, sx, s)
      if (nch <= 1) { SL_ROWSTAT_LAUNCH(1); }
      else if (nch == 2) { SL_ROWSTAT_LAUNCH(2); }
      else if (nch == 3) { SL_ROWSTAT_LAUNCH(3); }
      else { SL_ROWSTAT_LAUNCH(4); }
#undef SL_ROWSTAT_LAUNCH
      SL_CHECK_LAUNCH("gemm_stream_reduce(rowstat)");
      return 0;
    }
  }
  hipLaunchKernelGGL((gemm_stream_reduce_kernel<T, ACT>), dim3((unsigned)((threads + 255) / 256)), dim3(256), 0, st, p, sx, s);
  SL_CHECK_LAUNCH("gemm_stream_reduce");
  return 0;
}

template <typename T, int MT, int ACT, int RF, int NWV, int D, int NL>
static int launch_stream_cfg(GemmP& p, const SkinnyX& sx, const StreamX& s, hipStream_t st) {
  const int nfrag = (p.N + 15) / 16;
  const int nblocks = (nfrag + NWV * RF - 1) / (NWV * RF), mblocks = (p.M + MT * 16 - 1) / (MT * 16);
  dim3 grid((nblocks + 7) / 8 * 8 * mblocks, 1, s.splits);
  if (sx.fuse_rms != 0 && sx.rstd_in == nullptr)
    hipLaunchKernelGGL((gemm_stream_kernel<T, MT, ACT, RF, NWV, D, NL, true>), grid, dim3(64 * (NWV + NL)), 0, st, p, sx, s);
  else
    hipLaunchKernelGGL((gemm_stream_kernel<T, MT, ACT, RF, NWV, D, NL, false>), grid, dim3(64 * (NWV + NL)), 0, st, p, sx, s);
  SL_CHECK_LAUNCH("gemm_stream");
  return launch_stream_reduce<T, ACT>(p, sx, s, st);
}

template <typename T, int MT, int ACT>
static int launch_stream_mt(GemmP& p, const SkinnyX& sx, const StreamX& s, const StreamCfg& c, hipStream_t st) {
  if constexpr (sizeof(T) == 4) {
    return launch_stream_cfg<T, MT, ACT, 2, (MT > 8 ? 2 : 4), 2, (MT > 8 ? 2 : 1)>(p, sx, s, st);
  } else {
    if constexpr (MT > 8) {
      return launch_stream_cfg<T, MT, ACT, 2, 2, 4, 2>(p, sx, s, st);
    } else if constexpr (MT == 8) {
      if (c.nwv == 2) return launch_stream_cfg<T, MT, ACT, 2, 2, 4, 1>(p, sx, s, st);
      if (c.nl == 4) return launch_stream_cfg<T, MT, ACT, 2, 4, 4, 4>(p, sx, s, st);
      if (c.nl == 2) return launch_stream_cfg<T, MT, ACT, 2, 4, 4, 2>(p, sx, s, st);
      return launch_stream_cfg<T, MT, ACT, 2, 4, 4, 1>(p, sx, s, st);
    } else {
      if (c.nwv == 2) return launch_stream_cfg<T, MT, ACT, 2, 2, 4, 1>(p, sx, s, st);
      return launch_stream_cfg<T, MT, ACT, 2, 4, 4, 1>(p, sx, s, st);
    }
  }
}

template <typename T, int ACT>
static int launch_stream(GemmP& p, const SkinnyX& sx, const StreamX& s, const StreamCfg& c, hipStream_t st) {
  switch (c.mt) {
    case 2: return launch_stream_mt<T, 2, ACT>(p, sx, s, c, st);
    case 4: return launch_stream_mt<T, 4, ACT>(p, sx, s, c, st);
    case 8: return launch_stream_mt<T, 8, ACT>(p, sx, s, c, st);
    default: return launch_stream_mt<T, 16, ACT>(p, sx, s, c, st);
  }
}

template <typename T>
static int stream_typed(GemmP& p, const SkinnyX& sx, int act, const StreamX& s, const StreamCfg& c, hipStream_t st) {
  switch (act) {
    case SL_ACT_NONE: return launch_stream<T, SL_ACT_NONE>(p, sx, s, c, st);
    case SL_ACT_SILU_MUL: return launch_stream<T, SL_ACT_SILU_MUL>(p, sx, s, c, st);
    case SL_ACT_ROPE_KV:
      if constexpr (sizeof(T) == 2) { if (sx.kv8) return launch_stream<T, SL_ACT_ROPE_KV8>(p, sx, s, c, st); }
      return launch_stream<T, SL_ACT_ROPE_KV>(p, sx, s, c, st);
  }
  sl_set_error("sl_gemm: packed weights are not built with act %d for M > 16 streaming", act);
  return SL_ERR_UNSUPPORTED;
}

static bool stream_wide_ok(const SkinnyX& sx, int act, const StreamCfg& c, bool have_ws) {
  if (!c.wide || (sx.fuse_rms != 0 && sx.rstd_in == nullptr)) return false;
  if (act != SL_ACT_NONE && act != SL_ACT_SILU_MUL && act != SL_ACT_ROPE_KV) return false;
  return c.wsplits == 1 || have_ws;
}

template <typename T, int ACT>
static int launch_stream_wide_act(GemmP& p, const SkinnyX& sx, const StreamX& s, hipStream_t st) {
  const int nfrag = (p.N + 15) / 16, mblocks = (p.M + 255) / 256, nblocks = (nfrag + 7) / 8;
  constexpr int LDS_BYTES = 3 * (256 * TROWB + 8 * 2 * 1024);
  dim3 grid((nblocks + 7) / 8 * 8 * mblocks, 1, s.splits);
  static std::atomic<uint64_t> attr_set{0};
  int devid = 0;
  SL_HIP(hipGetDevice(&devid));
  if (devid < 0 || devid >= 64 || !((attr_set.load(std::memory_order_relaxed) >> devid) & 1)) {
    SL_HIP(hipFuncSetAttribute((const void*)gemm_stream_wide_kernel<T, ACT>, hipFuncAttributeMaxDynamicSharedMemorySize, LDS_BYTES));
    if (devid >= 0 && devid < 64) attr_set.fetch_or(1ull << devid, std::memory_order_relaxed);
  }
  hipLaunchKernelGGL((gemm_stream_wide_kernel<T, ACT>), grid, dim3(768), LDS_BYTES, st, p, sx, s);
  SL_CHECK_LAUNCH("gemm_stream_wide");
  if (s.cnt) return 0;
  return launch_stream_reduce<T, ACT>(p, sx, s, st);
}

template <typename T>
static int launch_stream_wide(GemmP& p, const SkinnyX& sx, int act, const StreamX& s, hipStream_t st) {
  switch (act) {
    case SL_ACT_SILU_MUL: return launch_stream_wide_act<T, SL_ACT_SILU_MUL>(p, sx, s, st);
    case SL_ACT_ROPE_KV:
      if constexpr (sizeof(T) == 2) { if (sx.kv8) return launch_stream_wide_act<T, SL_ACT_ROPE_KV8>(p, sx, s, st); }
      return launch_stream_wide_act<T, SL_ACT_ROPE_KV>(p, sx, s, st);
    default: return launch_stream_wide_act<T, SL_ACT_NONE>(p, sx, s, st);
  }
}

int sl_gemm_stream_launch(GemmP& p, const SkinnyX& sx, int dtype, int act, void* split_ws, size_t split_ws_bytes, hipStream_t st) {
  const int kstep = dtype == SL_F32 ? 16 : 32;
  SL_CHECK_ARG(p.K % (2 * kstep) == 0, "sl_gemm: streaming path needs K %% %d == 0 (K=%d)", 2 * kstep, p.K);
  StreamCfg c = stream_cfg(sl_family_rows(p.M), p.N, p.K, kstep, split_ws != nullptr, dtype);
  StreamX s;
  const bool wide = stream_wide_ok(sx, act, c, split_ws != nullptr);
  if (wide) c.splits = c.wsplits;

  s.np = (p.N + 15) / 16 * 16;
  const size_t per_split = ((size_t)p.M * s.np + (size_t)p.M) * sizeof(float);
  const size_t hdr = stream_ws_header(p.M);
  split_ws_bytes = (split_ws && split_ws_bytes > hdr) ? split_ws_bytes - hdr : 0;
  if (c.splits > 1 && (size_t)c.splits * per_split > split_ws_bytes) c.splits = (int)(split_ws_bytes / per_split);
  if (c.splits < 1) c.splits = 1;
  const int nst = p.K / (2 * kstep);
  s.sps = (nst + c.splits - 1) / c.splits;
  s.splits = (nst + s.sps - 1) / s.sps;
  c.splits = s.splits;
  SL_CHECK_ARG(sx.norm_out == nullptr || sx.rstd_out != nullptr, "sl_gemm: norm_out comes from the pass that forms rstd_out (pass both)");
  if (sx.rstd_out) {
    SL_CHECK_ARG(act == SL_ACT_NONE && (p.N + 15) / 16 * 4 <= 1024 && s.splits > 1,
                 "sl_gemm: rstd_out needs the plain epilogue, N <= 4096 and a K-split (splits=%d; see sl_gemm_split_count)", s.splits);
  }
  s.part = split_ws ? (float*)((unsigned char*)split_ws + hdr) : nullptr;
  s.part_ss = s.part ? s.part + (size_t)s.splits * p.M * s.np : nullptr;
  s.cnt = nullptr; s.ss_part = nullptr;
  if (wide && s.splits > 1 && sl_env().stream_fixup != 0 && sx.norm_out == nullptr) {
    const int nbv = ((p.N + 15) / 16 + 7) / 8, mbl = (p.M + 255) / 256;
    if (nbv * mbl <= 1024 && mbl <= 64 && (sx.rstd_out == nullptr || nbv <= 32)) {
      s.cnt = (int*)split_ws;
      s.ss_part = (float*)((unsigned char*)split_ws + 8192);
    }
  }
  if (dtype == SL_F32) return stream_typed<float>(p, sx, act, s, c, st);
  if (dtype == SL_F16) {
    if (wide) return launch_stream_wide<f16_t>(p, sx, act, s, st);
    return stream_typed<f16_t>(p, sx, act, s, c, st);
  }
  if (wide) return launch_stream_wide<bf16_t>(p, sx, act, s, st);
  return stream_typed<bf16_t>(p, sx, act, s, c, st);
}
```

### llm-speech-summarization_amd/csrc/runtime.hip

```cpp
#include <cmath>
#include <vector>

#include "common.h"
#include "gemm_internal.h"

int sl_attn_decode_impl(const void* q, int64_t q_stride, const void* k_cache, const void* v_cache, void* out, const int32_t* ctx_len,
                        int ctx_add, int32_t B, int32_t n_heads, int32_t n_kv, int32_t D, int32_t max_ctx, float scale, int32_t dtype,
                        hipStream_t st);
int sl_greedy_select_impl(const float* logits, int32_t B, int32_t V, const int32_t* eos_ids, int32_t n_eos, int32_t pad_id,
                          int32_t use_eos, int32_t advance_ctx, int32_t* unfinished, int32_t* ctx_len, int32_t* gen_count,
                          int32_t* finish_len, int32_t* next_ids, int32_t* out_ids, int32_t max_new, hipStream_t st, const int32_t* row_limit);
int sl_greedy_select_partial_impl(const float* amax_val, const int32_t* amax_idx, int32_t n_groups, int32_t B, const int32_t* eos_ids, int32_t n_eos,
                                  int32_t pad_id, int32_t use_eos, int32_t advance_ctx, int32_t* unfinished, int32_t* ctx_len, int32_t* gen_count,
                                  int32_t* finish_len, int32_t* next_ids, int32_t* out_ids, int32_t max_new, hipStream_t st, const int32_t* row_limit);
int sl_sample_select_impl(const float* logits, int32_t B, int32_t V, float temperature, int32_t top_k, float top_p, uint64_t seed,
                          const int32_t* eos_ids, int32_t n_eos, int32_t pad_id, int32_t use_eos, int32_t advance_ctx, int32_t* unfinished,
                          int32_t* ctx_len, int32_t* gen_count, int32_t* finish_len, int32_t* next_ids, int32_t* out_ids, int32_t max_new,
                          int32_t* choice_ws, hipStream_t st, const int32_t* row_limit, const int32_t* row_ids);

int sl_attn_decode_split_zero_counters(void* workspace, int B, int n_heads, int n_kv, int max_ctx, hipStream_t st);
int sl_attn_decode_split_impl(const void* q, int64_t q_stride, const void* k_cache, const void* v_cache, void* out, void* workspace,
                              const int32_t* ctx_len, int ctx_add, int32_t B, int32_t n_heads, int32_t n_kv, int32_t D, int32_t max_ctx,
                              float scale, int32_t dtype, hipStream_t st, int counters, int shared_prefix, int kv_format);
size_t sl_attn_decode_split_ws(int B, int n_heads, int n_kv, int max_ctx);
// ... 221 lines not shown
  }
  for (int i = 0; i < nc; ++i)
    for (int u = 0; u < n_utt; ++u) row0[i][u + 1] = row0[i][u] + Lc[i][u];
  std::vector<int64_t> desc((size_t)((nc - 1) * n_utt + n_utt * G) * 4);
  std::vector<int64_t> max_rows(nc, 0);
  for (int i = 1; i < nc; ++i)
    for (int u = 0; u < n_utt; ++u) {
      int64_t* d = &desc[(size_t)((i - 1) * n_utt + u) * 4];
      d[0] = Lc[i][u]; d[1] = row0[i - 1][u] * m->conv_dim[i - 1]; d[2] = row0[i][u] * m->conv_dim[i]; d[3] = 0;
      if (Lc[i][u] > max_rows[i]) max_rows[i] = Lc[i][u];
    }
  std::vector<int64_t> xg_off(n_utt + 1, 0);
  for (int u = 0; u < n_utt; ++u) xg_off[u + 1] = xg_off[u] + (pl.T[u] + kpos) * H;
  const size_t pos_desc0 = (size_t)(nc - 1) * n_utt * 4;
  for (int u = 0; u < n_utt; ++u)
    for (int g = 0; g < G; ++g) {
      int64_t* d = &desc[pos_desc0 + (size_t)(u * G + g) * 4];
      d[0] = pl.T[u]; d[1] = xg_off[u] + (int64_t)g * (pl.T[u] + kpos) * Hg; d[2] = pl.tok0[u] * H + (int64_t)g * Hg; d[3] = d[2];
    }
  {
    std::vector<int32_t> cu(n_utt + 1), kl(n_utt);
    for (int u = 0; u <= n_utt; ++u) cu[u] = (int32_t)pl.tok0[u];
    for (int u = 0; u < n_utt; ++u) kl[u] = (int32_t)pl.T[u];
    SL_HIP(hipMemcpyAsync(w.cu, cu.data(), (n_utt + 1) * sizeof(int32_t), hipMemcpyHostToDevice, st));
    SL_HIP(hipMemcpyAsync(w.cuk, cu.data(), n_utt * sizeof(int32_t), hipMemcpyHostToDevice, st));
    SL_HIP(hipMemcpyAsync(w.klen, kl.data(), n_utt * sizeof(int32_t), hipMemcpyHostToDevice, st));
    SL_HIP(hipMemcpyAsync(w.desc, desc.data(), desc.size() * sizeof(int64_t), hipMemcpyHostToDevice, st));
    std::vector<int64_t> prec;
    proj_records(m, pl, n_utt, out_ld, out_row_offsets_host, prec);
    SL_HIP(hipMemcpyAsync(w.pdesc, prec.data(), prec.size() * sizeof(int64_t), hipMemcpyHostToDevice, st));
    std::vector<int64_t> c0(2 * (size_t)(n_utt + 1));
    for (int u = 0; u <= n_utt; ++u) { c0[u] = sample_offsets_host[u] - sample_offsets_host[0]; c0[n_utt + 1 + u] = row0[0][u]; }
    SL_HIP(hipMemcpyAsync(w.c0desc, c0.data(), c0.size() * sizeof(int64_t), hipMemcpyHostToDevice, st));
    SL_HIP(hipStreamSynchronize(st));
  }
  void* cur = w.convA;
  {
    int64_t max_L0 = 0;
    for (int u = 0; u < n_utt; ++u) max_L0 = Lc[0][u] > max_L0 ? Lc[0][u] : max_L0;
    SL_TRY(sl_hubert_conv0_batch(waves + sample_offsets_host[0], w.c0desc, w.c0desc + n_utt + 1, n_utt, max_L0, m->conv0_w, m->conv0_b, m->conv0_g,
                                 m->conv0_beta, cur, m->conv_dim[0], m->conv_kernel[0], m->conv_stride[0], 1e-5f, dt, stream));
  }
  for (int i = 1; i < nc; ++i) {
    const int Cin = m->conv_dim[i - 1], Cout = m->conv_dim[i], k = m->conv_kernel[i], s = m->conv_stride[i];
    void* dst = (i == nc - 1) ? w.feat : (cur == w.convA ? w.convB : w.convA);
    sl_gemm_args a;
    memset(&a, 0, sizeof(a));
    a.A = cur; a.lda = (int64_t)s * Cin;
    a.W = m->conv_w[i]; a.ldw = (int64_t)k * Cin;
    a.C = dst; a.ldc = Cout; a.bias = m->conv_b[i];
    a.M = (int)max_rows[i]; a.N = Cout; a.K = k * Cin; a.batch = n_utt; a.dtype = dt; a.act = SL_ACT_NONE;
    sl_gemm_ex_args ex;
    memset(&ex, 0, sizeof(ex));
    ex.groups = w.desc + (size_t)(i - 1) * n_utt * 4; ex.w_mod = 1;
    SL_TRY(sl_gemm_impl(&a, nullptr, &ex, st));
    SL_TRY(sl_layernorm(dst, dst, m->conv_g[i], m->conv_beta[i], row0[i][n_utt], Cout, 1e-5f, 1, dt, stream));
    cur = dst;
  }
  const int NT = (int)pl.total_T;
  SL_TRY(sl_layernorm(w.feat, w.feat, m->fp_ln_g, m->fp_ln_b, NT, Cl, m->ln_eps, 0, dt, stream));
  SL_TRY(gemm(dt, w.feat, Cl, m->fp_w, Cl, w.x, H, m->fp_b, nullptr, 0, NT, H, Cl, SL_ACT_NONE, 0, st));
  {
    SL_TRY(sl_posconv_stage_batch(w.x, w.xg, w.cu, w.klen, n_utt, pl.max_T, H, G, kpos, dt, stream));
    sl_gemm_args a;
    memset(&a, 0, sizeof(a));
    a.A = w.xg; a.lda = Hg;
    a.W = m->pos_w; a.ldw = (int64_t)kpos * Hg; a.strideW = (int64_t)Hg * kpos * Hg;
    a.C = w.ln; a.ldc = H;
    a.bias = m->pos_b; a.strideBias = Hg;
    a.residual = w.x; a.ldr = H;
    a.M = (int)pl.max_T; a.N = Hg; a.K = kpos * Hg; a.batch = n_utt * G; a.dtype = dt; a.act = SL_ACT_GELU;
    sl_gemm_ex_args ex;
    memset(&ex, 0, sizeof(ex));
    ex.groups = w.desc + pos_desc0; ex.w_mod = G;
    SL_TRY(sl_gemm_impl(&a, nullptr, &ex, st));
    void* t = w.x; w.x = w.ln; w.ln = t;
  }
  return encoder_tail(m, w, pl, n_utt, out, out_ld, out_row_offsets_host, last_hidden, st);
}

static int whisper_plan(const sl_hubert_model* m, int n_utt, HubertPlan& pl) {
  const int64_t T = m->pos_k;
  pl.T.assign(n_utt, T); pl.P.resize(n_utt); pl.tok0.resize(n_utt + 1);
  SL_CHECK_ARG(T >= m->pool_kernel, "sl_whisper_forward: %lld frames < pool kernel %d", (long long)T, m->pool_kernel);
  for (int u = 0; u < n_utt; ++u) { pl.P[u] = (T - m->pool_kernel) / m->pool_stride + 1; pl.tok0[u] = (int64_t)u * T; pl.total_P += pl.P[u]; }
  pl.tok0[n_utt] = (int64_t)n_utt * T;
  pl.total_T = (int64_t)n_utt * T; pl.max_T = T;
  pl.max_conv_elems = (int64_t)n_utt * (2 * T + 2) * (m->hidden > m->conv_dim[0] ? m->hidden : m->conv_dim[0]);
  return 0;
}

extern "C" size_t sl_whisper_workspace_bytes(const sl_hubert_model* m, int32_t n_utt) {
  HubertPlan pl;
  if (whisper_plan(m, n_utt, pl) != 0) return 0;
  HubertWs w;
  return hubert_carve(m, pl, n_utt, nullptr, 0, w);
}

extern "C" int sl_whisper_forward(const sl_hubert_model* m, const void* mel, int32_t n_utt, void* out, int64_t out_ld,
                                  const int64_t* out_row_offsets_host, void* last_hidden, void* workspace, size_t workspace_bytes,
                                  sl_stream stream) {
  SL_CHECK_ARG(m && mel && workspace && n_utt > 0, "sl_whisper_forward: bad arguments");
  SL_CHECK_ARG(m->reserved == 1, "sl_whisper_forward: model struct is not a Whisper front end");
  SL_CHECK_ARG((m->proj_w && out) || (!m->proj_w && last_hidden), "sl_whisper_forward: need `out` (pool) or `last_hidden`");
  SL_CHECK_ARG(m->hidden % m->n_heads == 0 && m->hidden / m->n_heads == 64, "sl_whisper_forward: head_dim must be 64");
  hipStream_t st = (hipStream_t)stream;
  const int dt = m->dtype, H = m->hidden, n_mel = m->conv_dim[0];
  const size_t sz = sl_dtype_size(dt);
  const int64_t T = m->pos_k, F = 2 * T;
  HubertPlan pl;
  SL_TRY(whisper_plan(m, n_utt, pl));
  HubertWs w;
  const size_t need = hubert_carve(m, pl, n_utt, workspace, workspace_bytes, w);
  SL_CHECK_ARG(need <= workspace_bytes, "sl_whisper_forward: workspace %zu B < required %zu B", workspace_bytes, need);
  {
    std::vector<int32_t> cu(n_utt + 1), kl(n_utt, (int32_t)T);
    for (int u = 0; u <= n_utt; ++u) cu[u] = (int32_t)(u * T);
    SL_HIP(hipMemcpyAsync(w.cu, cu.data(), (n_utt + 1) * sizeof(int32_t), hipMemcpyHostToDevice, st));
    SL_HIP(hipMemcpyAsync(w.cuk, cu.data(), n_utt * sizeof(int32_t), hipMemcpyHostToDevice, st));
    SL_HIP(hipMemcpyAsync(w.klen, kl.data(), n_utt * sizeof(int32_t), hipMemcpyHostToDevice, st));
    std::vector<int64_t> prec;
    proj_records(m, pl, n_utt, out_ld, out_row_offsets_host, prec);
    SL_HIP(hipMemcpyAsync(w.pdesc, prec.data(), prec.size() * sizeof(int64_t), hipMemcpyHostToDevice, st));
    SL_HIP(hipStreamSynchronize(st));
  }
  SL_HIP(hipMemsetAsync(w.convA, 0, (size_t)n_utt * (F + 2) * n_mel * sz, st));
  SL_HIP(hipMemsetAsync(w.convB, 0, (size_t)n_utt * (F + 2) * H * sz, st));
  SL_HIP(hipMemcpy2DAsync(bptr(w.convA) + (size_t)n_mel * sz, (size_t)(F + 2) * n_mel * sz, mel, (size_t)F * n_mel * sz, (size_t)F * n_mel * sz, n_utt,
                          hipMemcpyDeviceToDevice, st));
  sl_gemm_args a;
  memset(&a, 0, sizeof(a));
  a.A = w.convA; a.lda = n_mel; a.strideA = (F + 2) * n_mel;
  a.W = m->conv_w[1]; a.ldw = 3 * n_mel;
  a.C = bptr(w.convB) + (size_t)H * sz; a.ldc = H; a.strideC = (F + 2) * H;
  a.bias = m->conv_b[1];
  a.M = (int)F; a.N = H; a.K = 3 * n_mel; a.batch = n_utt; a.dtype = dt; a.act = SL_ACT_GELU;
  SL_TRY(sl_gemm_impl(&a, nullptr, nullptr, st));
  memset(&a, 0, sizeof(a));
  a.A = w.convB; a.lda = 2 * (int64_t)H; a.strideA = (F + 2) * H;
  a.W = m->conv_w[2]; a.ldw = 3 * (int64_t)H;
  a.C = w.x; a.ldc = H; a.strideC = T * H;
  a.bias = m->conv_b[2];
  a.residual = m->pos_w; a.ldr = H; a.strideR = 0;
  a.M = (int)T; a.N = H; a.K = 3 * H; a.batch = n_utt; a.dtype = dt; a.act = SL_ACT_GELU;
  SL_TRY(sl_gemm_impl(&a, nullptr, nullptr, st));
  return encoder_tail(m, w, pl, n_utt, out, out_ld, out_row_offsets_host, last_hidden, st);
}


struct LlamaWs {
  void *h, *qkv, *att, *mid, *last, *part, *split;
  size_t split_bytes;
  float *rstd_a, *rstd_b;
  int32_t *tok_seq, *tok_pos, *cu, *cuk, *klen;
  int32_t* last_row;
};

static size_t llama_carve(const sl_llama_model* m, int64_t n_tok, int nseq, void* base, size_t cap, LlamaWs& w) {
  const size_t sz = sl_dtype_size(m->dtype);
  const int qkv_w = (m->n_heads + 2 * m->n_kv_heads) * m->head_dim;
  Carver c(base, cap);
  w.h = c.take(n_tok * m->hidden * sz);
  w.qkv = c.take(n_tok * qkv_w * sz);
  w.att = c.take(n_tok * (int64_t)m->n_heads * m->head_dim * sz);
  w.mid = c.take(n_tok * (int64_t)m->ffn * sz);
  w.last = c.take((size_t)nseq * m->hidden * sz);
  w.part = c.take(sl_attn_decode_split_ws(nseq, m->n_heads, m->n_kv_heads, m->rope_len));
  {
    size_t sb = 0;
    const int shapes[5][2] = {{qkv_w, m->hidden}, {m->hidden, m->n_heads * m->head_dim}, {2 * m->ffn, m->hidden}, {m->hidden, m->ffn}, {m->vocab, m->hidden}};
    for (auto& sh : shapes) {
      const size_t b = sl_gemm_split_workspace_bytes(nseq, sh[0], sh[1], m->dtype);
      if (b > sb) sb = b;
    }
    w.split_bytes = sb;
    w.split = c.take(sb);
  }
  w.rstd_a = (float*)c.take((size_t)nseq * sizeof(float));
  w.rstd_b = (float*)c.take((size_t)nseq * sizeof(float));
  w.tok_seq = (int32_t*)c.take(n_tok * sizeof(int32_t));
  w.tok_pos = (int32_t*)c.take(n_tok * sizeof(int32_t));
  w.cu = (int32_t*)c.take((nseq + 2) * sizeof(int32_t));
  w.cuk = (int32_t*)c.take((nseq + 1) * sizeof(int32_t));
  w.klen = (int32_t*)c.take((nseq + 1) * sizeof(int32_t));
  w.last_row = (int32_t*)c.take((size_t)nseq * sizeof(int32_t));
  return c.off + 256;
}

extern "C" size_t sl_llama_workspace_bytes(const sl_llama_model* m, int64_t n_tok, int32_t nseq) {
  LlamaWs w;
  return llama_carve(m, n_tok, nseq, nullptr, 0, w);
}

static int llama_check(const sl_llama_model* m, const sl_kv_cache* kv) {
  SL_CHECK_ARG(m && kv && m->layers && m->embed && m->lm_head && m->final_norm && m->rope_cos && m->rope_sin, "llama: null model field");
  if (kv->reserved != SL_KV_MODEL_DTYPE) SL_TRY(sl_kv_format_check("llama (sl_kv_cache.reserved)", kv->reserved, m->dtype, m->head_dim));
  SL_CHECK_ARG(m->head_dim == 128, "llama: head_dim %d not built (128)", m->head_dim);
  SL_CHECK_ARG(kv->k_cache && kv->v_cache && kv->slots > 0 && kv->max_ctx > 0, "llama: bad kv cache");
  SL_CHECK_ARG(kv->shared_prefix >= 0 && kv->shared_prefix <= kv->max_ctx, "llama: kv cache shared_prefix %d outside [0, max_ctx=%d]", kv->shared_prefix, kv->max_ctx);
  SL_CHECK_ARG(kv->max_ctx <= m->rope_len, "llama: max_ctx %d exceeds the rope table (%d)", kv->max_ctx, m->rope_len);
  return 0;
}

static int llama_wdec_check(const char* who, const sl_llama_model* m, int rows) {
  if (m->reserved == SL_WDEC_MODEL_DTYPE) return 0;
  SL_CHECK_ARG(m->reserved == SL_WDEC_E4M3, "%s: unknown decode-weight format %d (sl_llama_model.reserved: 0 = model dtype, 1 = e4m3 weight images)", who, m->reserved);
  if (m->dtype == SL_F32) {
    sl_set_error("%s: e4m3 decode weights are built for bf16 / fp16 models, not float32 (the parity mode)", who);
    return SL_ERR_UNSUPPORTED;
  }
  SL_CHECK_ARG(m->dec_fused_norm == 1 && m->lm_head_dec, "%s: e4m3 decode weights need dec_fused_norm = 1 and lm_head_dec", who);
  for (int l = 0; l < m->n_layers; ++l) {
    const sl_llama_layer& L = m->layers[l];
    SL_CHECK_ARG(L.wqkv_dec && L.wo_dec && L.wgu_dec && L.wdown_dec, "%s: e4m3 decode weights: layer %d has a null *_dec image", who, l);
  }
  const int ks[3] = {m->hidden, m->n_heads * m->head_dim, m->ffn};
  for (int k : ks)
    if (k % 64 != 0) {
      sl_set_error("%s: e4m3 decode weights need every reduction length to be a multiple of 64 (hidden=%d, n_heads*head_dim=%d, ffn=%d)", who, ks[0], ks[1], ks[2]);
      return SL_ERR_UNSUPPORTED;
    }
  if (sl_family_rows(rows) > sl_w8_max_rows()) {
    sl_set_error("%s: e4m3 decode weights run up to sl_w8_max_rows() = %d rows per decode step, not %d (use the 16-bit decode copies)", who, sl_w8_max_rows(), sl_family_rows(rows));
    return SL_ERR_UNSUPPORTED;
  }
  return 0;
}

static inline size_t kv_elem_bytes(const sl_llama_model* m, const sl_kv_cache* kv) { return sl_kv_elem_size(kv->reserved, m->dtype); }
static inline size_t kv_layer_bytes(const sl_llama_model* m, const sl_kv_cache* kv) {
  return (size_t)kv->slots * m->n_kv_heads * kv->max_ctx * m->head_dim * kv_elem_bytes(m, kv);
}

extern "C" size_t sl_kv_cache_bytes(const sl_llama_model* m, int32_t slots, int32_t max_ctx, int32_t kv_format) {
  if (!m || slots <= 0 || max_ctx <= 0 || m->n_layers <= 0) { sl_set_error("sl_kv_cache_bytes: bad arguments"); return 0; }
  if (sl_kv_format_check("sl_kv_cache_bytes", kv_format, m->dtype, m->head_dim) != 0) return 0;
  return (size_t)m->n_layers * slots * m->n_kv_heads * max_ctx * m->head_dim * sl_kv_elem_size(kv_format, m->dtype);
}

__global__ __launch_bounds__(256) void gather_rows_kernel(const uint4* __restrict__ src, uint4* __restrict__ dst, const int32_t* __restrict__ map,
                                                          int64_t n_rows, int row_vec) {
  const int64_t i = (int64_t)blockIdx.x * 256 + threadIdx.x;
  if (i >= n_rows * row_vec) return;
  const int64_t r = i / row_vec;
  const int c = (int)(i - r * row_vec);
  dst[i] = src[(int64_t)map[r] * row_vec + c];
}
static int gather_rows(const void* src, void* dst, const int32_t* map, int64_t n_rows, size_t row_bytes, hipStream_t st) {
  const int row_vec = (int)(row_bytes / 16);
  hipLaunchKernelGGL(gather_rows_kernel, dim3((unsigned)((n_rows * row_vec + 255) / 256)), dim3(256), 0, st, (const uint4*)src, (uint4*)dst, map, n_rows, row_vec);
  SL_CHECK_LAUNCH("gather_rows");
  return 0;
}
__global__ __launch_bounds__(64) void kv_prefix_broadcast_kernel(uint4* __restrict__ kc, uint4* __restrict__ vc, int nkv, int max_ctx, int row_vec) {
  const int pos = blockIdx.x, h = blockIdx.y, s = blockIdx.z + 1;
  uint4* c = threadIdx.x < 32 ? kc : vc;
  const int lane = threadIdx.x & 31;
  if (lane >= row_vec) return;
  const int64_t src = ((int64_t)h * max_ctx + pos) * row_vec + lane;
  c[((int64_t)s * nkv * max_ctx) * row_vec + src] = c[src];
}

__global__ __launch_bounds__(256) void weight_prefetch_kernel(const uint4* __restrict__ w, size_t n16, uint32_t* __restrict__ sink) {
  uint32_t acc = 0;
  const size_t stride = (size_t)gridDim.x * 256;
  size_t i = (size_t)blockIdx.x * 256 + threadIdx.x;
  for (; i + 7 * stride < n16; i += 8 * stride) {
    uint4 v[8];
#pragma unroll
    for (int u = 0; u < 8; ++u) v[u] = w[i + u * stride];
#pragma unroll
    for (int u = 0; u < 8; ++u) acc ^= v[u].x ^ v[u].y ^ v[u].z ^ v[u].w;
  }
  for (; i < n16; i += stride) { const uint4 v = w[i]; acc ^= v.x ^ v.y ^ v.z ^ v.w; }
  if (acc == 0x9e3779b9u && sink) *sink = acc;
}

struct DecodePrefetch {
  hipStream_t main = nullptr, side = nullptr;
  hipEvent_t ev = nullptr;
  uint32_t* sink = nullptr;
  bool on = false;
  int ahead(const void* next, size_t bytes) {
    if (!on || !next || bytes < (1u << 20)) return 0;
    SL_HIP(hipEventRecord(ev, main));
    SL_HIP(hipStreamWaitEvent(side, ev, 0));
    const size_t n16 = bytes / 16;
    int blocks = (int)((n16 + 256 * 8 - 1) / (256 * 8));
    blocks = blocks > 512 ? 512 : (blocks < 1 ? 1 : blocks);
    hipLaunchKernelGGL(weight_prefetch_kernel, dim3(blocks), dim3(256), 0, side, (const uint4*)next, n16, sink);
    SL_CHECK_LAUNCH("weight_prefetch");
    return 0;
  }
  int join() {
    if (!on) return 0;
    SL_HIP(hipEventRecord(ev, side));
    SL_HIP(hipStreamWaitEvent(main, ev, 0));
    return 0;
  }
};
static thread_local DecodePrefetch* g_prefetch = nullptr;

static int dec_gemm(const sl_llama_model* m, const LlamaWs& w, const void* A, int64_t lda, const void* Wp, void* C, int64_t ldc, const void* res,
                    int M, int N, int K, int act, int out_f32, const sl_gemm_fused* fx_in, hipStream_t st, const float* rstd_in = nullptr,
                    float* rstd_out = nullptr, void* norm_out = nullptr, const void* norm_gain = nullptr) {
  sl_gemm_fused fxl;
  if (fx_in) fxl = *fx_in; else memset(&fxl, 0, sizeof(fxl));
  fxl.split_ws = w.split; fxl.split_ws_bytes = w.split_bytes;
  fxl.rstd_in = rstd_in; fxl.rstd_out = rstd_out; fxl.rms_eps = m->rms_eps;
  fxl.norm_out = norm_out; fxl.norm_gain = norm_gain;
  const sl_gemm_fused* fx = &fxl;
  sl_gemm_args a;
  memset(&a, 0, sizeof(a));
  a.A = A; a.lda = lda; a.W = Wp; a.ldw = K; a.C = C; a.ldc = ldc; a.residual = res; a.ldr = ldc;
  a.M = M; a.N = N; a.K = K; a.batch = 1; a.dtype = m->dtype; a.act = act; a.out_f32 = out_f32;
  a.w_layout = m->reserved == SL_WDEC_E4M3 ? SL_W_PACKED_E4M3 : SL_W_PACKED;
  return sl_gemm_impl(&a, fx, nullptr, st);
}

static int llama_layer(const sl_llama_model* m, const sl_kv_cache* kv, int l, void* x, int64_t n, LlamaWs& w, bool decode, int nseq,
                       int max_qlen, const int32_t* ctx_len_dev, hipStream_t st, bool rstd_chain = false, const float* rstd_qkv = nullptr,
                       int prefix_bcast = 0, int bcast_slots = 0, bool rstd_pass = false, const int32_t* tail_rows = nullptr, int n_tail = 0) {
  const sl_llama_layer& L = m->layers[l];
  const int dt = m->dtype, H = m->hidden, D = m->head_dim, nh = m->n_heads, nkv = m->n_kv_heads;
  const int qkv_w = (nh + 2 * nkv) * D;
  void* kc = bptr(kv->k_cache) + (size_t)l * kv_layer_bytes(m, kv);
  void* vc = bptr(kv->v_cache) + (size_t)l * kv_layer_bytes(m, kv);
  const float scale = 1.0f / sqrtf((float)D);
  if (decode && L.wqkv_dec && L.wo_dec && L.wgu_dec && L.wdown_dec) {
    sl_gemm_fused fx;
    memset(&fx, 0, sizeof(fx));
    fx.fuse_rms = m->dec_fused_norm; fx.rms_eps = m->rms_eps;
    fx.rope_cos = m->rope_cos; fx.rope_sin = m->rope_sin; fx.tok_pos = ctx_len_dev; fx.tok_seq = w.tok_seq;
    fx.k_cache = kc; fx.v_cache = vc; fx.n_heads = nh; fx.n_kv_heads = nkv; fx.max_ctx = kv->max_ctx; fx.reserved = kv->reserved;
    DecodePrefetch* pf = g_prefetch;
    const size_t esz = sl_dtype_size(dt);
    const bool w8 = m->reserved == SL_WDEC_E4M3;
    const size_t b_qkv = w8 ? sl_w8_image_bytes(qkv_w, H) : (size_t)qkv_w * H * esz, b_o = w8 ? sl_w8_image_bytes(H, nh * D) : (size_t)H * nh * D * esz,
                 b_gu = w8 ? sl_w8_image_bytes(2 * m->ffn, H) : (size_t)2 * m->ffn * H * esz, b_down = w8 ? sl_w8_image_bytes(H, m->ffn) : (size_t)H * m->ffn * esz;
    const sl_llama_layer* Ln = (l + 1 < m->n_layers) ? &m->layers[l + 1] : nullptr;
    if (pf && l == 0) { SL_TRY(pf->ahead(L.wqkv_dec, b_qkv)); SL_TRY(pf->ahead(L.wo_dec, b_o)); }
    if (pf) SL_TRY(pf->ahead(L.wgu_dec, b_gu));
    const void* a_in = x;
    if (!m->dec_fused_norm) { SL_TRY(sl_rmsnorm(x, w.h, L.norm1, n, H, m->rms_eps, dt, (sl_stream)st)); a_in = w.h; }
    if (rstd_pass) { SL_TRY(sl_rmsnorm_rstd_impl(x, nullptr, nullptr, w.rstd_b, n, H, m->rms_eps, dt, st)); rstd_qkv = w.rstd_b; }
    SL_TRY(dec_gemm(m, w, a_in, H, L.wqkv_dec, w.qkv, (int64_t)nh * D, nullptr, (int)n, qkv_w, H, SL_ACT_ROPE_KV, 0, &fx, st, rstd_qkv));
    SL_TRY(sl_attn_decode_split_impl(w.qkv, (int64_t)nh * D, kc, vc, w.att, w.part, ctx_len_dev, 1, (int)n, nh, nkv, D, kv->max_ctx, scale, dt, st, 1, kv->shared_prefix, kv->reserved));
    if (pf) SL_TRY(pf->ahead(L.wdown_dec, b_down));
    if (rstd_pass) {
      SL_TRY(dec_gemm(m, w, w.att, (int64_t)nh * D, L.wo_dec, x, H, x, (int)n, H, nh * D, SL_ACT_NONE, 0, nullptr, st));
      if (L.wgu && sl_env().decode_tiled) {
        SL_TRY(sl_rmsnorm(x, w.h, L.norm2, n, H, m->rms_eps, dt, (sl_stream)st));
        SL_TRY(gemm(dt, w.h, H, L.wgu, H, w.mid, m->ffn, nullptr, nullptr, 0, (int)n, 2 * m->ffn, H, SL_ACT_SILU_MUL, 0, st));
      } else {
        SL_TRY(sl_rmsnorm_rstd_impl(x, nullptr, nullptr, w.rstd_a, n, H, m->rms_eps, dt, st));
        sl_gemm_fused fn;
        memset(&fn, 0, sizeof(fn));
        fn.fuse_rms = 1; fn.rms_eps = m->rms_eps;
        SL_TRY(dec_gemm(m, w, x, H, L.wgu_dec, w.mid, m->ffn, nullptr, (int)n, 2 * m->ffn, H, SL_ACT_SILU_MUL, 0, &fn, st, w.rstd_a));
      }
    } else if (sl_family_rows((int)n) > 896 && sl_is16(dt) && L.wgu && rstd_chain && sl_env().decode_tiled) {
      SL_TRY(dec_gemm(m, w, w.att, (int64_t)nh * D, L.wo_dec, x, H, x, (int)n, H, nh * D, SL_ACT_NONE, 0, nullptr, st, nullptr, w.rstd_a, w.h, L.norm2));
      SL_TRY(gemm(dt, w.h, H, L.wgu, H, w.mid, m->ffn, nullptr, nullptr, 0, (int)n, 2 * m->ffn, H, SL_ACT_SILU_MUL, 0, st));
    } else {
      SL_TRY(dec_gemm(m, w, w.att, (int64_t)nh * D, L.wo_dec, x, H, x, (int)n, H, nh * D, SL_ACT_NONE, 0, nullptr, st, nullptr,
                      rstd_chain ? w.rstd_a : nullptr));
      sl_gemm_fused fn;
      memset(&fn, 0, sizeof(fn));
      fn.fuse_rms = m->dec_fused_norm; fn.rms_eps = m->rms_eps;
      a_in = x;
      if (pf && Ln) SL_TRY(pf->ahead(Ln->wqkv_dec, b_qkv));
      if (!m->dec_fused_norm) { SL_TRY(sl_rmsnorm(x, w.h, L.norm2, n, H, m->rms_eps, dt, (sl_stream)st)); a_in = w.h; }
      SL_TRY(dec_gemm(m, w, a_in, H, L.wgu_dec, w.mid, m->ffn, nullptr, (int)n, 2 * m->ffn, H, SL_ACT_SILU_MUL, 0, &fn, st,
                      rstd_chain ? w.rstd_a : nullptr));
    }
    if (pf && Ln) SL_TRY(pf->ahead(Ln->wo_dec, b_o));
    SL_TRY(dec_gemm(m, w, w.mid, m->ffn, L.wdown_dec, x, H, x, (int)n, H, m->ffn, SL_ACT_NONE, 0, nullptr, st, nullptr,
                    rstd_chain ? w.rstd_b : nullptr));
    return 0;
  }
  SL_TRY(sl_rmsnorm(x, w.h, L.norm1, n, H, m->rms_eps, dt, (sl_stream)st));
  SL_TRY(gemm(dt, w.h, H, L.wqkv, H, w.qkv, qkv_w, nullptr, nullptr, 0, (int)n, qkv_w, H, SL_ACT_NONE, 0, st));
  SL_TRY(sl_rope_kv_append_ex(w.qkv, kc, vc, w.tok_seq, decode ? ctx_len_dev : w.tok_pos, m->rope_cos, m->rope_sin, n, nh, nkv, D, kv->max_ctx,
                              dt, kv->reserved, (sl_stream)st));
  if (decode) {
    SL_TRY(sl_attn_decode_split_impl(w.qkv, qkv_w, kc, vc, w.att, w.part, ctx_len_dev, 1, (int)n, nh, nkv, D, kv->max_ctx, scale, dt, st, 1, kv->shared_prefix, kv->reserved));
  } else {
    if (prefix_bcast > 0 && bcast_slots > 1) {
      const int row_vec = (int)(D * kv_elem_bytes(m, kv) / 16);
      SL_CHECK_ARG(row_vec <= 32 && (D * kv_elem_bytes(m, kv)) % 16 == 0, "llama: shared prefix broadcast needs K / V rows of <= 512 bytes");
      hipLaunchKernelGGL(kv_prefix_broadcast_kernel, dim3(prefix_bcast, nkv, bcast_slots - 1), dim3(64), 0, st, (uint4*)kc, (uint4*)vc, nkv, kv->max_ctx, row_vec);
      SL_CHECK_LAUNCH("kv_prefix_broadcast");
    }
    sl_attn_args a;
    memset(&a, 0, sizeof(a));
    a.q = w.qkv; a.q_row_stride = qkv_w; a.q_head_stride = D;
    a.k = kc; a.k_row_stride = D; a.k_head_stride = (int64_t)kv->max_ctx * D;
    a.v = vc; a.v_row_stride = D; a.v_head_stride = (int64_t)kv->max_ctx * D;
    a.out = w.att; a.o_row_stride = (int64_t)nh * D; a.o_head_stride = D;
    a.cu_q = w.cu; a.cu_k = w.cuk; a.klen = w.klen;
    if (kv->reserved == SL_KV_FP8_E4M3) {
      const size_t esz = sl_dtype_size(dt);
      a.k = bptr(w.qkv) + (size_t)nh * D * esz; a.k_row_stride = qkv_w; a.k_head_stride = D;
      a.v = bptr(w.qkv) + (size_t)(nh + nkv) * D * esz; a.v_row_stride = qkv_w; a.v_head_stride = D;
      a.cu_k = w.cu;
    }
    a.nseq = nseq; a.max_qlen = max_qlen; a.n_heads = nh; a.n_kv_heads = nkv; a.head_dim = D; a.causal = 1; a.dtype = dt; a.scale = scale;
    SL_TRY(sl_attn_fwd(&a, (sl_stream)st));
  }
  if (tail_rows && !decode) {
    const size_t esz = sl_dtype_size(dt);
    void* att_t = w.qkv;
    SL_TRY(gather_rows(w.att, att_t, tail_rows, n_tail, (size_t)nh * D * esz, st));
    SL_TRY(gather_rows(x, w.last, tail_rows, n_tail, (size_t)H * esz, st));
    SlFamilyPin pin((int)n);
    SL_TRY(gemm(dt, att_t, (int64_t)nh * D, L.wo, (int64_t)nh * D, w.last, H, nullptr, w.last, H, n_tail, H, nh * D, SL_ACT_NONE, 0, st));
    SL_TRY(sl_rmsnorm(w.last, w.h, L.norm2, n_tail, H, m->rms_eps, dt, (sl_stream)st));
    SL_TRY(gemm(dt, w.h, H, L.wgu, H, w.mid, m->ffn, nullptr, nullptr, 0, n_tail, 2 * m->ffn, H, SL_ACT_SILU_MUL, 0, st));
    SL_TRY(gemm(dt, w.mid, m->ffn, L.wdown, m->ffn, w.last, H, nullptr, w.last, H, n_tail, H, m->ffn, SL_ACT_NONE, 0, st));
    return 0;
  }
  SL_TRY(gemm(dt, w.att, (int64_t)nh * D, L.wo, (int64_t)nh * D, x, H, nullptr, x, H, (int)n, H, nh * D, SL_ACT_NONE, 0, st));
  SL_TRY(sl_rmsnorm(x, w.h, L.norm2, n, H, m->rms_eps, dt, (sl_stream)st));
  SL_TRY(gemm(dt, w.h, H, L.wgu, H, w.mid, m->ffn, nullptr, nullptr, 0, (int)n, 2 * m->ffn, H, SL_ACT_SILU_MUL, 0, st));
  SL_TRY(gemm(dt, w.mid, m->ffn, L.wdown, m->ffn, x, H, nullptr, x, H, (int)n, H, m->ffn, SL_ACT_NONE, 0, st));
  return 0;
}

static int llama_prefill_impl(const sl_llama_model* m, const sl_kv_cache* kv, void* x, const int32_t* cu_seqlens_host, int32_t nseq,
                              float* logits, int32_t* ctx_len_dev, void* hidden_taps, void* workspace, size_t workspace_bytes,
                              sl_stream stream, int slot_stride) {
  SL_TRY(llama_check(m, kv));
  SL_CHECK_ARG(x && cu_seqlens_host && logits && ctx_len_dev && workspace && nseq > 0 && slot_stride >= 1 && (int64_t)nseq * slot_stride <= kv->slots,
               "sl_llama_prefill: bad arguments");
  hipStream_t st = (hipStream_t)stream;
  const int64_t n_tok = cu_seqlens_host[nseq];
  const int dt = m->dtype, H = m->hidden;
  const size_t sz = sl_dtype_size(dt);
  LlamaWs w;
  const size_t need = llama_carve(m, n_tok, nseq, workspace, workspace_bytes, w);
  SL_CHECK_ARG(need <= workspace_bytes, "sl_llama_prefill: workspace %zu B < required %zu B", workspace_bytes, need);
  SL_CHECK_ARG(((size_t)H * sz) % 16 == 0, "sl_llama_prefill: hidden rows must be a multiple of 16 bytes");
  std::vector<int32_t> tseq(n_tok), tpos(n_tok), cuk(nseq + 1), kl(nseq + 1), ctx(nseq), cuq(nseq + 2), last_row(nseq);
  int max_q = 0;
  int P = (kv->shared_prefix > 0 && nseq > 1 && !hidden_taps && sl_env().prefill_share_prefix && kv->reserved != SL_KV_FP8_E4M3 && slot_stride == 1) ? kv->shared_prefix : 0;
  for (int s = 0; s < nseq; ++s) {
    const int len = cu_seqlens_host[s + 1] - cu_seqlens_host[s];
    SL_CHECK_ARG(len > 0 && len <= kv->max_ctx, "sl_llama_prefill: sequence %d length %d outside (0, max_ctx=%d]", s, len, kv->max_ctx);
    SL_CHECK_ARG(kv->shared_prefix <= len, "sl_llama_prefill: kv cache shared_prefix %d exceeds sequence %d (%d tokens)", kv->shared_prefix, s, len);
    if (len <= P) P = 0;
  }
  int64_t n_run = n_tok;
  int nseq_attn = nseq;
  if (P > 0) {
    std::vector<int32_t> map;
    map.reserve(n_tok);
    for (int t = 0; t < P; ++t) { map.push_back(cu_seqlens_host[0] + t); }
    cuq[0] = 0; cuq[1] = P; cuk[0] = 0; kl[0] = P;
    for (int t = 0; t < P; ++t) { tseq[t] = 0; tpos[t] = t; }
    max_q = P;
    for (int s = 0; s < nseq; ++s) {
      const int len = cu_seqlens_host[s + 1] - cu_seqlens_host[s], tail = len - P;
      const int r0 = (int)map.size();
      for (int t = 0; t < tail; ++t) { map.push_back(cu_seqlens_host[s] + P + t); tseq[r0 + t] = s; tpos[r0 + t] = P + t; }
      cuq[s + 2] = r0 + tail;
      cuk[s + 1] = s * m->n_kv_heads * kv->max_ctx;
      kl[s + 1] = len; ctx[s] = len;
      last_row[s] = r0 + tail - 1;
      if (tail > max_q) max_q = tail;
    }
    n_run = (int64_t)map.size();
    nseq_attn = nseq + 1;
    SL_HIP(hipMemcpyAsync(w.tok_pos, map.data(), n_run * sizeof(int32_t), hipMemcpyHostToDevice, st));
    SL_TRY(gather_rows(x, w.mid, w.tok_pos, n_run, (size_t)H * sz, st));
    SL_HIP(hipMemcpyAsync(x, w.mid, (size_t)n_run * H * sz, hipMemcpyDeviceToDevice, st));
    SL_HIP(hipStreamSynchronize(st));
  } else {
    for (int s = 0; s < nseq; ++s) {
      const int len = cu_seqlens_host[s + 1] - cu_seqlens_host[s];
      for (int t = 0; t < len; ++t) { tseq[cu_seqlens_host[s] + t] = s * slot_stride; tpos[cu_seqlens_host[s] + t] = t; }
      cuk[s] = s * slot_stride * m->n_kv_heads * kv->max_ctx;
      kl[s] = len; ctx[s] = len;
      cuq[s] = cu_seqlens_host[s];
      last_row[s] = cu_seqlens_host[s + 1] - 1;
      if (len > max_q) max_q = len;
    }
    cuq[nseq] = cu_seqlens_host[nseq];
  }
  SL_HIP(hipMemcpyAsync(w.tok_seq, tseq.data(), n_run * sizeof(int32_t), hipMemcpyHostToDevice, st));
  SL_HIP(hipMemcpyAsync(w.tok_pos, tpos.data(), n_run * sizeof(int32_t), hipMemcpyHostToDevice, st));
  SL_HIP(hipMemcpyAsync(w.cu, cuq.data(), (nseq_attn + 1) * sizeof(int32_t), hipMemcpyHostToDevice, st));
  SL_HIP(hipMemcpyAsync(w.cuk, cuk.data(), nseq_attn * sizeof(int32_t), hipMemcpyHostToDevice, st));
  SL_HIP(hipMemcpyAsync(w.klen, kl.data(), nseq_attn * sizeof(int32_t), hipMemcpyHostToDevice, st));
  SL_HIP(hipMemcpyAsync(ctx_len_dev, ctx.data(), nseq * sizeof(int32_t), hipMemcpyHostToDevice, st));
  SL_HIP(hipMemcpyAsync(w.last_row, last_row.data(), nseq * sizeof(int32_t), hipMemcpyHostToDevice, st));
  SL_HIP(hipStreamSynchronize(st));
  const bool prune = !hidden_taps && m->n_layers > 0 && sl_env().prefill_prune_last != 0;
  for (int l = 0; l < m->n_layers; ++l) {
    if (hidden_taps) SL_HIP(hipMemcpyAsync(bptr(hidden_taps) + (size_t)l * n_tok * H * sz, x, n_tok * H * sz, hipMemcpyDeviceToDevice, st));
    const bool tail = prune && l == m->n_layers - 1;
    SL_TRY(llama_layer(m, kv, l, x, n_run, w, false, nseq_attn, max_q, nullptr, st, false, nullptr, P, nseq, false, tail ? w.last_row : nullptr, nseq));
  }
  if (hidden_taps) {
    SL_TRY(sl_rmsnorm(x, bptr(hidden_taps) + (size_t)m->n_layers * n_tok * H * sz, m->final_norm, n_tok, H, m->rms_eps, dt, stream));
  }
  if (!prune) SL_TRY(gather_rows(x, w.last, w.last_row, nseq, (size_t)H * sz, st));
  SL_TRY(sl_rmsnorm(w.last, w.last, m->final_norm, nseq, H, m->rms_eps, dt, stream));
  SL_TRY(gemm(dt, w.last, H, m->lm_head, H, logits, m->vocab, nullptr, nullptr, 0, nseq, m->vocab, H, SL_ACT_NONE, 1, st));
  return 0;
}

extern "C" int sl_llama_prefill(const sl_llama_model* m, const sl_kv_cache* kv, void* x, const int32_t* cu_seqlens_host, int32_t nseq,
                                float* logits, int32_t* ctx_len_dev, void* hidden_taps, void* workspace, size_t workspace_bytes,
// ... 665 lines not shown
```

Before: 68960.

## Add 128-row fill streaming GEMM form with split RMSNorm partial sums for large decode batches

Adds a new warp-specialized streaming GEMM kernel (DMA waves plus MMA waves, 128-row by 6 or 10 fragment blocks). It is picked by a cost model when the existing narrow or wide forms would underfill the CUs or need split-K reduction. For the o-proj to gate/up step at large family rows, the o-proj kernel writes per-column-block partial sums of squares. The following SILU_MUL GEMM epilogue then reduces those partials into rstd and applies it, so no separate rstd computation is needed. This adds kernel variants, an added heuristic, and workspace for the partials, and it applies only to large decode batches.

```diff
diff --git a/llm-speech-summarization_amd/csrc/api.hip b/llm-speech-summarization_amd/csrc/api.hip
--- a/llm-speech-summarization_amd/csrc/api.hip
+++ b/llm-speech-summarization_amd/csrc/api.hip
@@ -102,6 +102,7 @@
   e.stream_wide = env_int("SL_STREAM_WIDE", 1);
   e.stream_wsplits = env_int("SL_STREAM_WSPLITS", 0);
   e.stream_fixup = env_int("SL_STREAM_FIXUP", 0);
+  e.stream_fill = env_int("SL_STREAM_FILL", 1);
   const char* sc = getenv("SL_STREAM_CFG");
   if (sc && sc[0]) {
     int sp = 0, nwv = 0, mt = 0;
diff --git a/llm-speech-summarization_amd/csrc/common.h b/llm-speech-summarization_amd/csrc/common.h
--- a/llm-speech-summarization_amd/csrc/common.h
+++ b/llm-speech-summarization_amd/csrc/common.h
@@ -372,6 +372,7 @@
   int stream_wide;
   int stream_wsplits;
   int stream_fixup;
+  int stream_fill;
   int stream_nl;
 };
 const SlEnv& sl_env();
diff --git a/llm-speech-summarization_amd/csrc/gemm.hip b/llm-speech-summarization_amd/csrc/gemm.hip
--- a/llm-speech-summarization_amd/csrc/gemm.hip
+++ b/llm-speech-summarization_amd/csrc/gemm.hip
@@ -964,7 +964,7 @@
 
 template <typename T>
 static int gemm_typed(const sl_gemm_args* a, GemmP& p, const SkinnyX& sx, hipStream_t st, void* sk_ws, size_t sk_ws_bytes, const SlEnv& e) {
-  const bool skinny = sl_family_rows(a->M) <= 64 && !p.ta && !p.tw && !p.res_f32 && !p.grp && no_rider(p) && !p.post && !p.colsum;
+  const bool skinny = sl_family_rows(a->M) <= 64 && !p.ta && !p.tw && !p.res_f32 && !p.grp && no_rider(p) && !p.post && !p.colsum && !p.rs_part;
   const bool packed = a->w_layout == SL_W_PACKED;
   if (!skinny && (packed || a->act == SL_ACT_ROPE_KV || sx.fuse_rms)) {
     sl_set_error("sl_gemm: packed weights / ROPE_KV / fused RMSNorm need plain operands (no transposes / groups), M=%d", a->M);
@@ -989,7 +989,9 @@
   }
 }
 
-int sl_gemm_impl(const sl_gemm_args* a, const sl_gemm_fused* fx, const sl_gemm_ex_args* ex, hipStream_t st) {
+int sl_gemm_impl(const sl_gemm_args* a, const sl_gemm_fused* fx, const sl_gemm_ex_args* ex, hipStream_t st) { return sl_gemm_impl_rows(a, fx, ex, nullptr, st); }
+
+int sl_gemm_impl_rows(const sl_gemm_args* a, const sl_gemm_fused* fx, const sl_gemm_ex_args* ex, const SlGemmRows* rows, hipStream_t st) {
   SL_CHECK_ARG(a != nullptr, "sl_gemm: null args");
   const SlEnv& e = sl_env();
   SL_CHECK_ARG(a->M > 0 && a->N > 0 && a->K > 0 && a->batch > 0, "sl_gemm: bad shape M=%d N=%d K=%d batch=%d", a->M, a->N, a->K, a->batch);
@@ -1092,7 +1094,19 @@
     sx.cos = fx->rope_cos; sx.sin = fx->rope_sin; sx.pos = fx->tok_pos; sx.seq = fx->tok_seq;
     sx.kc = fx->k_cache; sx.vc = fx->v_cache; sx.nh = fx->n_heads; sx.nkv = fx->n_kv_heads; sx.max_ctx = fx->max_ctx;
     sx.rstd_in = fx->rstd_in; sx.rstd_out = fx->rstd_out; sx.norm_out = fx->norm_out; sx.norm_gain = fx->norm_gain;
-    SL_CHECK_ARG((!fx->norm_out && !fx->norm_gain) || (fx->norm_out && fx->norm_gain && fx->rstd_out && !a->out_f32), "sl_gemm: norm_out needs norm_gain, rstd_out and an output in the storage type");
+    SL_CHECK_ARG((!fx->norm_out && !fx->norm_gain) || (fx->norm_out && fx->norm_gain && (fx->rstd_out || (rows && rows->ss_part_out)) && !a->out_f32),
+                 "sl_gemm: norm_out needs norm_gain, rstd_out and an output in the storage type");
+  }
+  if (rows && rows->ss_part_out) {
+    SL_CHECK_ARG(a->w_layout == SL_W_PACKED && a->act == SL_ACT_NONE && sl_is16(a->dtype) && !a->out_f32 && !a->bias && !ex && a->batch == 1 && !(fx && fx->rstd_out),
+                 "sl_gemm: ss_part_out needs one plain 16-bit product on packed weights, without bias or rstd_out");
+    sx.ss_part = rows->ss_part_out;
+  }
+  if (rows && rows->rs_part) {
+    SL_CHECK_ARG(a->w_layout == SL_W_ROWMAJOR && a->act == SL_ACT_SILU_MUL && sl_is16(a->dtype) && !ex && a->batch == 1 && rows->rs_nparts > 0 &&
+                     rows->rs_nparts <= SL_SS_PARTS && rows->rs_n > 0,
+                 "sl_gemm: rs_part needs one row-major 16-bit SILU_MUL product and 1 .. %d partial sums per row", SL_SS_PARTS);
+    p.rs_part = rows->rs_part; p.rs_nparts = rows->rs_nparts; p.rs_n = rows->rs_n; p.rs_eps = rows->rs_eps;
   }
   if (a->act == SL_ACT_ROPE_KV) {
     SL_CHECK_ARG(fx && fx->rope_cos && fx->rope_sin && fx->tok_pos && fx->tok_seq && fx->k_cache && fx->v_cache,
@@ -1102,8 +1116,10 @@
     sx.kv8 = fx->reserved == SL_KV_FP8_E4M3;
   }
   if (a->w_layout == SL_W_PACKED && sl_family_rows(a->M) > e.stream_min_m && a->batch == 1 && !ex && a->act != SL_ACT_GELU &&
-      a->K % slab_elems(a->dtype) == 0)
+      a->K % slab_elems(a->dtype) == 0) {
+    if (e.gemm_log) sl_gemm_stream_log(p, sx, a->dtype, a->act, fx && fx->split_ws);
     return e.gemm_log == 2 ? 0 : sl_gemm_stream_launch(p, sx, a->dtype, a->act, fx ? fx->split_ws : nullptr, fx ? fx->split_ws_bytes : 0, st);
+  }
   SL_CHECK_ARG(a->w_layout != SL_W_PACKED || sl_family_rows(a->M) <= 64, "sl_gemm: packed weights with M=%d > 64 need batch 1 and K %% 64 == 0", a->M);
   if (w8) {
     SL_CHECK_ARG(a->act >= SL_ACT_NONE && a->act <= SL_ACT_ROPE_KV, "sl_gemm: unknown act %d", a->act);
@@ -1140,6 +1156,13 @@
   return sl_gemm_impl(a, nullptr, ex, (hipStream_t)stream);
 }
 
+extern "C" int sl_gemm_rows_internal(const sl_gemm_args* a, const sl_gemm_fused* fx, float* ss_part_out, const float* rs_part, int32_t rs_nparts, int32_t rs_n,
+                                     float rs_eps, sl_stream stream) {
+  SlGemmRows rows = {};
+  rows.ss_part_out = ss_part_out; rows.rs_part = rs_part; rows.rs_nparts = rs_nparts; rows.rs_n = rs_n; rows.rs_eps = rs_eps;
+  return sl_gemm_impl_rows(a, fx, nullptr, &rows, (hipStream_t)stream);
+}
+
 extern "C" int sl_gemm_fused_decode(const sl_gemm_args* a, const sl_gemm_fused* fx, sl_stream stream) {
   SL_CHECK_ARG(fx != nullptr, "sl_gemm_fused_decode: null fused args");
   return sl_gemm_impl(a, fx, nullptr, (hipStream_t)stream);
diff --git a/llm-speech-summarization_amd/csrc/gemm_epilogue.h b/llm-speech-summarization_amd/csrc/gemm_epilogue.h
--- a/llm-speech-summarization_amd/csrc/gemm_epilogue.h
+++ b/llm-speech-summarization_amd/csrc/gemm_epilogue.h
@@ -58,18 +58,37 @@
   if constexpr (ACT == SL_ACT_SILU_MUL) {
     static_assert(NT % 2 == 0, "gate/up fragments come in pairs");
     const int nout = p.N >> 1;
+    constexpr int NH = (MT * 16 + 63) / 64;
+    const bool rsc = p.rs_part != nullptr;
+    float rsl[NH];
+    if (rsc) {
+#pragma unroll
+      for (int h = 0; h < NH; ++h) {
+        int row = row_base + h * 64 + q * 16 + r;
+        row = row < p.M ? row : p.M - 1;
+        float t = 0.f;
+        for (int j = 0; j < p.rs_nparts; ++j) t += p.rs_part[(int64_t)j * p.M + row];
+        rsl[h] = rsqrtf(t / (float)p.rs_n + p.rs_eps);
+      }
+    }
 #pragma unroll
     for (int pr = 0; pr < NT / 2; ++pr) {
       const int gcol = col0 + (2 * pr) * 16, ucol = gcol + 16;
       const int ocol = (col_base >> 1) + pr * 16 + r;
-      if (ocol >= nout) continue;
-      const float bg = bias ? to_f32(bias[gcol]) : 0.f, bu = bias ? to_f32(bias[ucol]) : 0.f;
+      if (!rsc && ocol >= nout) continue;
+      const bool live = ocol < nout;
+      const float bg = bias && live ? to_f32(bias[gcol]) : 0.f, bu = bias && live ? to_f32(bias[ucol]) : 0.f;
 #pragma unroll
       for (int m = 0; m < MT; ++m)
 #pragma unroll
         for (int i = 0; i < 4; ++i) {
           const int row = row0 + m * 16 + i;
-          if (row < p.M) store_out<T>(p, Cb, Rb, row, ocol, silu(acc[m][2 * pr][i] + bg) * (acc[m][2 * pr + 1][i] + bu));
+          float g = acc[m][2 * pr][i], u = acc[m][2 * pr + 1][i];
+          if (rsc) {
+            const float sc = __shfl(rsl[m >> 2], (m & 3) * 16 + q * 4 + i, 64);
+            g *= sc; u *= sc;
+          }
+          if (live && row < p.M) store_out<T>(p, Cb, Rb, row, ocol, silu(g + bg) * (u + bu));
         }
     }
   } else {
diff --git a/llm-speech-summarization_amd/csrc/gemm_internal.h b/llm-speech-summarization_amd/csrc/gemm_internal.h
--- a/llm-speech-summarization_amd/csrc/gemm_internal.h
+++ b/llm-speech-summarization_amd/csrc/gemm_internal.h
@@ -35,6 +35,9 @@
   int32_t* defer;
   int krun;
   uint32_t* stamp;
+  const float* rs_part;
+  int rs_nparts, rs_n;
+  float rs_eps;
 };
 
 __device__ __forceinline__ bool resolve_group(GemmP& p, int z, int bm, int64_t& a_off, int& wz, int tile_rows = 128) {
@@ -147,7 +150,17 @@
   float* rstd_out;
   void* norm_out;
   const void* norm_gain;
+  float* ss_part;
 };
+constexpr int SL_SS_PARTS = 32;
+struct SlGemmRows {
+  float* ss_part_out;
+  const float* rs_part;
+  int rs_nparts, rs_n;
+  float rs_eps;
+};
+int sl_gemm_impl_rows(const sl_gemm_args* a, const sl_gemm_fused* fx, const sl_gemm_ex_args* ex, const SlGemmRows* rows, hipStream_t st);
+int sl_gemm_stream_fill_bf(int M, int N, int K, int dtype);
 constexpr int SL_ACT_ROPE_KV8 = 64 + SL_ACT_ROPE_KV;
 constexpr bool sl_act_is_rope_kv(int act) { return act == SL_ACT_ROPE_KV || act == SL_ACT_ROPE_KV8; }
 template <typename T>
@@ -162,3 +175,4 @@
 int sl_gemm_stream_launch(GemmP& p, const SkinnyX& sx, int dtype, int act, void* split_ws, size_t split_ws_bytes, hipStream_t st);
 size_t sl_gemm_stream_ws_bytes(int M, int N, int K, int dtype);
 int sl_gemm_stream_splits(int M, int N, int K, int dtype);
+void sl_gemm_stream_log(const GemmP& p, const SkinnyX& sx, int dtype, int act, bool have_ws);
diff --git a/llm-speech-summarization_amd/csrc/gemm_stream.hip b/llm-speech-summarization_amd/csrc/gemm_stream.hip
--- a/llm-speech-summarization_amd/csrc/gemm_stream.hip
+++ b/llm-speech-summarization_amd/csrc/gemm_stream.hip
@@ -548,6 +548,202 @@
   }
 }
 
+template <typename T, int ACT, int BF, int NS>
+__global__ __launch_bounds__(768) void gemm_stream_fill_kernel(GemmP p, SkinnyX sx, StreamX s) {
+  constexpr int VEC = Vec16<T>::VEC;
+  constexpr int KSTEP = MMA<T>::KSTEP;
+  constexpr int CW = 8;
+  constexpr int BM = 128, MTW = 2, RFW = BF / 2;
+  static_assert(BF % 2 == 0, "two column waves");
+  constexpr bool PAIRS = sl_act_is_rope_kv(ACT);
+  static_assert(ACT == SL_ACT_NONE || PAIRS, "plain and RoPE / KV-append epilogues");
+  static_assert(!PAIRS || RFW % 2 == 1, "the pair hand-off below is written for an odd fragment count per wave");
+  constexpr int SLAB_X = BM * TROWB, SLAB_W = BF * 2 * 1024, SLOT = SLAB_X + SLAB_W;
+  constexpr int NXD = BM / 32, NWD = BF / 2;
+  constexpr int NDMA = NXD + NWD;
+  extern __shared__ __attribute__((aligned(16))) unsigned char smem[];
+  __shared__ f32x4 xch[PAIRS ? 4 * MTW * 64 : 1];
+
+  const int tid = threadIdx.x, lane = tid & 63;
+  const int wave = __builtin_amdgcn_readfirstlane(tid >> 6);
+  const int r = lane & 15, q = lane >> 4;
+  const int mblocks = (p.M + BM - 1) / BM;
+  const int nfrag = (p.N + 15) >> 4;
+  const int xj = blockIdx.x >> 3, nb = (xj / mblocks) * 8 + (blockIdx.x & 7);
+  if (nb * BF >= nfrag) return;
+  const int m0 = (xj % mblocks) * BM;
+  const int nks = p.K / KSTEP;
+  const int n_it = nks >> 1;
+  const int g_last = n_it - 1;
+  const int wm = (wave >> 1) & 3, wn = wave & 1;
+  const int mw = m0 + wm * (MTW * 16), fi0 = nb * BF + wn * RFW;
+
+  f32x4 acc[RFW][MTW];
+#pragma unroll
+  for (int t = 0; t < MTW; ++t)
+#pragma unroll
+    for (int f = 0; f < RFW; ++f) acc[f][t] = f32x4{0.f, 0.f, 0.f, 0.f};
+
+  if (wave >= CW) {
+    const int lw = wave - CW;
+    const T* A = (const T*)p.A;
+    const T* W = (const T*)p.W;
+    const int ch = (lane & 7) ^ ((lane >> 3) & 7);
+    const T* gx[NXD];
+#pragma unroll
+    for (int i = 0; i < NXD; ++i) {
+      int xr_ = m0 + lw * 32 + (lane >> 3) + 8 * i; xr_ = xr_ < p.M ? xr_ : p.M - 1;
+      gx[i] = A + (int64_t)xr_ * p.lda + ch * VEC;
+    }
+    const T* gw[NWD];
+#pragma unroll
+    for (int i = 0; i < NWD; ++i) {
+      const int j = lw * NWD + i;
+      int fi = nb * BF + (j >> 1); fi = fi < nfrag ? fi : nfrag - 1;
+      gw[i] = W + (int64_t)fi * nks * (64 * VEC) + (int64_t)(j & 1) * (64 * VEC) + lane * VEC;
+    }
+    unsigned char* xbase = smem + lw * (32 * TROWB);
+    unsigned char* wbase = smem + SLAB_X + lw * (NWD * 1024);
+    auto dma = [&](int it) {
+      const int stg = it < g_last ? it : g_last;
+      const int so = (it % NS) * SLOT;
+#pragma unroll
+      for (int i = 0; i < NXD; ++i)
+        __builtin_amdgcn_global_load_lds((glb_ptr_t)(gx[i] + (int64_t)stg * (2 * KSTEP)), (lds_ptr_t)(xbase + so + i * 1024), 16, 0, 0);
+#pragma unroll
+      for (int i = 0; i < NWD; ++i)
+        __builtin_amdgcn_global_load_lds((glb_ptr_t)(gw[i] + (int64_t)stg * (2 * 64 * VEC)), (lds_ptr_t)(wbase + so + i * 1024), 16, 0, 0);
+    };
+#pragma unroll
+    for (int i = 0; i < NS - 1; ++i) dma(i);
+    asm volatile("s_waitcnt vmcnt(%0)" ::"n"((NS - 2) * NDMA) : "memory");
+    __builtin_amdgcn_s_barrier();
+    for (int it = 0; it < n_it; ++it) {
+      dma(it + NS - 1);
+      asm volatile("s_waitcnt vmcnt(%0)" ::"n"((NS - 2) * NDMA) : "memory");
+      __builtin_amdgcn_s_barrier();
+    }
+    asm volatile("s_waitcnt vmcnt(0)" ::: "memory");
+  } else {
+    uint4 fx[2][MTW], fw[2][RFW];
+    auto rd = [&](int it, int s2, int set) {
+      const unsigned char* sl_ = smem + (it % NS) * SLOT;
+#pragma unroll
+      for (int t = 0; t < MTW; ++t) fx[set][t] = *(const uint4*)(sl_ + lds_off(wm * (MTW * 16) + t * 16 + r, s2 * 4 + q));
+#pragma unroll
+      for (int f = 0; f < RFW; ++f) fw[set][f] = *(const uint4*)(sl_ + SLAB_X + ((wn * RFW + f) * 2 + s2) * 1024 + lane * 16);
+    };
+    auto mma = [&](int set) {
+#pragma unroll
+      for (int t = 0; t < MTW; ++t)
+#pragma unroll
+        for (int f = 0; f < RFW; ++f) MMA<T>::step(acc[f][t], fw[set][f], fx[set][t]);
+#pragma unroll
+      for (int i = 0; i < MTW + RFW; ++i) {
+        __builtin_amdgcn_sched_group_barrier(0x008, 1, 0);
+        __builtin_amdgcn_sched_group_barrier(0x100, 1, 0);
+      }
+    };
+    __builtin_amdgcn_s_barrier();
+    rd(0, 0, 0);
+    for (int it = 0; it < n_it; ++it) {
+      __builtin_amdgcn_sched_barrier(0);
+      rd(it, 1, 1);
+      mma(0);
+      __builtin_amdgcn_sched_barrier(0);
+      asm volatile("s_waitcnt lgkmcnt(0)" ::: "memory");
+      __builtin_amdgcn_s_barrier();
+      rd(it + 1, 0, 0);
+      mma(1);
+      __builtin_amdgcn_sched_barrier(0);
+    }
+  }
+  if constexpr (!PAIRS) {
+    if (sx.ss_part == nullptr) {
+      if (wave < CW) {
+        float ssum[MTW] = {0.f, 0.f};
+        stream_finish<T, MTW, ACT, RFW>(p, sx, s, acc, ssum, false, mw, 0, fi0, nfrag, false, q, r);
+      }
+      return;
+    }
+    __shared__ float fl_ss[4][2][MTW * 16];
+    if (wave < CW) {
+      const T* gain = (const T*)sx.norm_gain;
+#pragma unroll
+      for (int t = 0; t < MTW; ++t) {
+        const int m = mw + t * 16 + r;
+        float sq = 0.f;
+        if (m < p.M) {
+#pragma unroll
+          for (int f = 0; f < RFW; ++f) {
+            const int col = (fi0 + f) * 16 + 4 * q;
+            float v[4];
+#pragma unroll
+            for (int i = 0; i < 4; ++i) v[i] = acc[f][t][i];
+            if (p.res) {
+              const uint2 rr = *(const uint2*)((const T*)p.res + (int64_t)m * p.ldr + col);
+              const f32x2_t lo = unpack2<T>(rr.x), hi = unpack2<T>(rr.y);
+              v[0] += lo.x; v[1] += lo.y; v[2] += hi.x; v[3] += hi.y;
+            }
+            const uint32_t plo = pack2<T>(v[0], v[1]), phi = pack2<T>(v[2], v[3]);
+            *(uint2*)((T*)p.C + (int64_t)m * p.ldc + col) = make_uint2(plo, phi);
+            const f32x2_t s01 = unpack2<T>(plo), s23 = unpack2<T>(phi);
+            v[0] = s01.x; v[1] = s01.y; v[2] = s23.x; v[3] = s23.y;
+#pragma unroll
+            for (int i = 0; i < 4; ++i) sq = fmaf(v[i], v[i], sq);
+            if (sx.norm_out) {
+              const uint2 gg = *(const uint2*)(gain + col);
+              const f32x2_t g01 = unpack2<T>(gg.x), g23 = unpack2<T>(gg.y);
+              *(uint2*)((T*)sx.norm_out + (int64_t)m * p.N + col) = make_uint2(pack2<T>(g01.x * v[0], g01.y * v[1]), pack2<T>(g23.x * v[2], g23.y * v[3]));
+            }
+          }
+        }
+        sq += __shfl_xor(sq, 16);
+        sq += __shfl_xor(sq, 32);
+        if (q == 0) fl_ss[wm][wn][t * 16 + r] = sq;
+      }
+    }
+    __syncthreads();
+    if (tid < BM) {
+      const int m = m0 + tid;
+      if (m < p.M) sx.ss_part[(int64_t)nb * p.M + m] = fl_ss[tid / (MTW * 16)][0][tid % (MTW * 16)] + fl_ss[tid / (MTW * 16)][1][tid % (MTW * 16)];
+    }
+  } else {
+    if (wave < CW && wn == 1) {
+#pragma unroll
+      for (int t = 0; t < MTW; ++t) xch[(wm * MTW + t) * 64 + lane] = acc[0][t];
+    }
+    __syncthreads();
+    if (wave >= CW) return;
+#pragma unroll
+    for (int t = 0; t < MTW; ++t) {
+      const int m = mw + t * 16 + r;
+      if (m >= p.M) continue;
+      const float rs = sx.rstd_in ? sx.rstd_in[m] : 1.0f;
+      float a[4], b[4];
+      if (wn == 0) {
+#pragma unroll
+        for (int pr = 0; pr < RFW / 2; ++pr) {
+#pragma unroll
+          for (int i = 0; i < 4; ++i) { a[i] = acc[2 * pr][t][i] * rs; b[i] = acc[2 * pr + 1][t][i] * rs; }
+          stream_epilogue4<T, ACT>(p, sx, m, fi0 + 2 * pr, 4 * q, a, b);
+        }
+        const f32x4 hi = xch[(wm * MTW + t) * 64 + lane];
+#pragma unroll
+        for (int i = 0; i < 4; ++i) { a[i] = acc[RFW - 1][t][i] * rs; b[i] = hi[i] * rs; }
+        stream_epilogue4<T, ACT>(p, sx, m, fi0 + RFW - 1, 4 * q, a, b);
+      } else {
+#pragma unroll
+        for (int pr = 0; pr < RFW / 2; ++pr) {
+#pragma unroll
+          for (int i = 0; i < 4; ++i) { a[i] = acc[2 * pr + 1][t][i] * rs; b[i] = acc[2 * pr + 2][t][i] * rs; }
+          stream_epilogue4<T, ACT>(p, sx, m, fi0 + 2 * pr + 1, 4 * q, a, b);
+        }
+      }
+    }
+  }
+}
+
 template <int UN, int NCH, bool PAIRS>
 __device__ __forceinline__ void reduce_add_splits(const float* rec, int64_t split_stride, int sp0, const uint32_t (&voff)[NCH], f32x4 (&a4)[NCH],
                                                   f32x4 (&b4)[NCH]) {
@@ -804,7 +1000,7 @@
   }
 }
 
-struct StreamCfg { int mt, splits, nwv, d, nl; int wide, wsplits; };
+struct StreamCfg { int mt, splits, nwv, d, nl; int wide, wsplits; int fill; };
 
 static StreamCfg stream_cfg(int M, int N, int K, int kstep, bool have_ws, int dtype) {
   StreamCfg c;
@@ -844,6 +1040,23 @@
       if (ws_ > 1) { c.wide = 1; c.wsplits = ws_; }
     }
   }
+  c.fill = 0;
+  if (sl_is16(dtype) && sl_env().stream_fill != 0) {
+    const int cus = 256;
+    const int today = c.wide ? ((M + 255) / 256) * ((nfrag + 7) / 8) : base;
+    const int today_splits = c.wide ? c.wsplits : c.splits;
+    const bool today_weak = today_splits > 1 || today * 10 < cus * 7;
+    const double cu_rate = 58.9e3, reduce_rate = 3.7e6;
+    const double today_rows = c.wide ? 256 + 128 : c.mt * 16 + c.nwv * 32;
+    const double t_today = (double)((nst + today_splits - 1) / today_splits) * today_rows * 128 / cu_rate +
+                           (today_splits > 1 ? (double)today_splits * M * N * 8 / reduce_rate : 0.0);
+    for (int bf = 10; bf >= 6 && !c.fill; bf -= 4) {
+      if (N % (16 * bf) != 0) continue;
+      const int blocks = ((M + 127) / 128) * (N / (16 * bf));
+      const double t_fill = (double)nst * (128 + 16 * bf) * 128 / cu_rate;
+      if (sl_env().stream_fill == 2 || (blocks * 10 >= cus * 9 && blocks <= cus && today_weak && t_fill <= 0.9 * t_today)) c.fill = bf;
+    }
+  }
   return c;
 }
 
@@ -860,6 +1073,11 @@
   const int most = c.wide && c.wsplits > c.splits ? c.wsplits : c.splits;
   size_t splits = most > 1 ? (size_t)most : 0;
   return stream_ws_header(M) + splits * ((size_t)M * np + (size_t)M) * sizeof(float) + 256;
+}
+
+int sl_gemm_stream_fill_bf(int M, int N, int K, int dtype) {
+  if (!sl_is16(dtype) || K % 64 != 0 || sl_env().stream_fill == 3) return 0;
+  return stream_cfg(sl_family_rows(M), N, K, 32, true, dtype).fill;
 }
 
 template <typename T, int ACT>
@@ -982,11 +1200,71 @@
   }
 }
 
+static bool stream_fill_ok(const SkinnyX& sx, const GemmP& p, int act, const StreamCfg& c) {
+  if (!c.fill || (sx.fuse_rms != 0 && sx.rstd_in == nullptr) || sx.rstd_out || (sx.norm_out && !sx.ss_part)) return false;
+  if ((sl_env().stream_fill == 3 && act != SL_ACT_ROPE_KV) || (sl_env().stream_fill == 4 && act != SL_ACT_NONE)) return false;
+  if (sx.ss_part) {
+    const uintptr_t al = 7;
+    if (act != SL_ACT_NONE || sx.rstd_in || p.bias || p.out_f32 || p.res_f32 || (p.ldc & 3) || (p.ldr & 3) || ((uintptr_t)p.C & al) || ((uintptr_t)p.res & al) ||
+        ((uintptr_t)sx.norm_out & al) || ((uintptr_t)sx.norm_gain & al) || p.N / (16 * c.fill) > SL_SS_PARTS)
+      return false;
+  }
+  return act == SL_ACT_NONE || act == SL_ACT_ROPE_KV;
+}
+
+template <typename T, int ACT, int BF>
+static int launch_stream_fill_act(GemmP& p, const SkinnyX& sx, const StreamX& s, hipStream_t st) {
+  constexpr int NS = 4;
+  constexpr int LDS_BYTES = NS * (128 * TROWB + BF * 2 * 1024);
+  const int nfrag = (p.N + 15) / 16, mblocks = (p.M + 127) / 128, nblocks = nfrag / BF;
+  dim3 grid((nblocks + 7) / 8 * 8 * mblocks, 1, 1);
+  static std::atomic<uint64_t> attr_set{0};
+  int devid = 0;
+  SL_HIP(hipGetDevice(&devid));
+  if (devid < 0 || devid >= 64 || !((attr_set.load(std::memory_order_relaxed) >> devid) & 1)) {
+    SL_HIP(hipFuncSetAttribute((const void*)gemm_stream_fill_kernel<T, ACT, BF, NS>, hipFuncAttributeMaxDynamicSharedMemorySize, LDS_BYTES));
+    if (devid >= 0 && devid < 64) attr_set.fetch_or(1ull << devid, std::memory_order_relaxed);
+  }
+  hipLaunchKernelGGL((gemm_stream_fill_kernel<T, ACT, BF, NS>), grid, dim3(768), LDS_BYTES, st, p, sx, s);
+  SL_CHECK_LAUNCH("gemm_stream_fill");
+  return 0;
+}
+
+template <typename T>
+static int launch_stream_fill(GemmP& p, const SkinnyX& sx, int act, int bf, const StreamX& s, hipStream_t st) {
+  if (act == SL_ACT_ROPE_KV) {
+    if (sx.kv8) return bf == 10 ? launch_stream_fill_act<T, SL_ACT_ROPE_KV8, 10>(p, sx, s, st) : launch_stream_fill_act<T, SL_ACT_ROPE_KV8, 6>(p, sx, s, st);
+    return bf == 10 ? launch_stream_fill_act<T, SL_ACT_ROPE_KV, 10>(p, sx, s, st) : launch_stream_fill_act<T, SL_ACT_ROPE_KV, 6>(p, sx, s, st);
+  }
+  return bf == 10 ? launch_stream_fill_act<T, SL_ACT_NONE, 10>(p, sx, s, st) : launch_stream_fill_act<T, SL_ACT_NONE, 6>(p, sx, s, st);
+}
+
+void sl_gemm_stream_log(const GemmP& p, const SkinnyX& sx, int dtype, int act, bool have_ws) {
+  const int kstep = dtype == SL_F32 ? 16 : 32;
+  if (p.K % (2 * kstep) != 0) return;
+  const StreamCfg c = stream_cfg(sl_family_rows(p.M), p.N, p.K, kstep, have_ws, dtype);
+  const int nfrag = (p.N + 15) / 16;
+  const char* form; int bm, bf, splits;
+  if (stream_fill_ok(sx, p, act, c)) { form = "fill"; bm = 128; bf = c.fill; splits = 1; }
+  else if (stream_wide_ok(sx, act, c, have_ws)) { form = "wide"; bm = 256; bf = 8; splits = c.wsplits; }
+  else { form = "narrow"; bm = c.mt * 16; bf = c.nwv * 2; splits = c.splits; }
+  const int blocks = ((p.M + bm - 1) / bm) * ((nfrag + bf - 1) / bf);
+  fprintf(stderr, "SLSTREAM fam=%d form=%s bm=%d bf=%d splits=%d blocks=%d\n", sl_family_rows(p.M), form, bm, bf, splits, blocks * splits);
+}
+
 int sl_gemm_stream_launch(GemmP& p, const SkinnyX& sx, int dtype, int act, void* split_ws, size_t split_ws_bytes, hipStream_t st) {
   const int kstep = dtype == SL_F32 ? 16 : 32;
   SL_CHECK_ARG(p.K % (2 * kstep) == 0, "sl_gemm: streaming path needs K %% %d == 0 (K=%d)", 2 * kstep, p.K);
   StreamCfg c = stream_cfg(sl_family_rows(p.M), p.N, p.K, kstep, split_ws != nullptr, dtype);
   StreamX s;
+  if (stream_fill_ok(sx, p, act, c)) {
+    memset(&s, 0, sizeof(s));
+    s.splits = 1; s.sps = p.K / (2 * kstep); s.np = (p.N + 15) / 16 * 16;
+    if (dtype == SL_F16) return launch_stream_fill<f16_t>(p, sx, act, c.fill, s, st);
+    return launch_stream_fill<bf16_t>(p, sx, act, c.fill, s, st);
+  }
+  SL_CHECK_ARG(sx.ss_part == nullptr, "sl_gemm: ss_part_out is written by the unsplit 128-row fill form only (M=%d N=%d K=%d: SL_STREAM_FILL, N %% 96 / 160, "
+               "<= %d column blocks, aligned 16-bit rows)", p.M, p.N, p.K, SL_SS_PARTS);
   const bool wide = stream_wide_ok(sx, act, c, split_ws != nullptr);
   if (wide) c.splits = c.wsplits;
 
diff --git a/llm-speech-summarization_amd/csrc/runtime.hip b/llm-speech-summarization_amd/csrc/runtime.hip
--- a/llm-speech-summarization_amd/csrc/runtime.hip
+++ b/llm-speech-summarization_amd/csrc/runtime.hip
@@ -397,6 +397,7 @@
   void *h, *qkv, *att, *mid, *last, *part, *split;
   size_t split_bytes;
   float *rstd_a, *rstd_b;
+  float* ss_part;
   int32_t *tok_seq, *tok_pos, *cu, *cuk, *klen;
   int32_t* last_row;
 };
@@ -423,6 +424,7 @@
   }
   w.rstd_a = (float*)c.take((size_t)nseq * sizeof(float));
   w.rstd_b = (float*)c.take((size_t)nseq * sizeof(float));
+  w.ss_part = (float*)c.take((size_t)SL_SS_PARTS * nseq * sizeof(float));
   w.tok_seq = (int32_t*)c.take(n_tok * sizeof(int32_t));
   w.tok_pos = (int32_t*)c.take(n_tok * sizeof(int32_t));
   w.cu = (int32_t*)c.take((nseq + 2) * sizeof(int32_t));
@@ -604,6 +606,25 @@
         fn.fuse_rms = 1; fn.rms_eps = m->rms_eps;
         SL_TRY(dec_gemm(m, w, x, H, L.wgu_dec, w.mid, m->ffn, nullptr, (int)n, 2 * m->ffn, H, SL_ACT_SILU_MUL, 0, &fn, st, w.rstd_a));
       }
+    } else if (sl_family_rows((int)n) > 896 && sl_is16(dt) && L.wgu && rstd_chain && sl_env().decode_tiled && !w8 && m->dec_fused_norm &&
+               sl_gemm_stream_fill_bf((int)n, H, nh * D, dt) && H / (16 * sl_gemm_stream_fill_bf((int)n, H, nh * D, dt)) <= SL_SS_PARTS && H % 4 == 0) {
+      sl_gemm_fused fo;
+      memset(&fo, 0, sizeof(fo));
+      fo.rms_eps = m->rms_eps; fo.norm_out = w.h; fo.norm_gain = L.norm2;
+      fo.split_ws = w.split; fo.split_ws_bytes = w.split_bytes;
+      sl_gemm_args a;
+      memset(&a, 0, sizeof(a));
+      a.A = w.att; a.lda = (int64_t)nh * D; a.W = L.wo_dec; a.ldw = nh * D; a.C = x; a.ldc = H; a.residual = x; a.ldr = H;
+      a.M = (int)n; a.N = H; a.K = nh * D; a.batch = 1; a.dtype = dt; a.act = SL_ACT_NONE; a.w_layout = SL_W_PACKED;
+      SlGemmRows ro = {};
+      ro.ss_part_out = w.ss_part;
+      SL_TRY(sl_gemm_impl_rows(&a, &fo, nullptr, &ro, st));
+      memset(&a, 0, sizeof(a));
+      a.A = w.h; a.lda = H; a.W = L.wgu; a.ldw = H; a.C = w.mid; a.ldc = m->ffn;
+      a.M = (int)n; a.N = 2 * m->ffn; a.K = H; a.batch = 1; a.dtype = dt; a.act = SL_ACT_SILU_MUL; a.w_layout = SL_W_ROWMAJOR;
+      SlGemmRows rg = {};
+      rg.rs_part = w.ss_part; rg.rs_nparts = H / (16 * sl_gemm_stream_fill_bf((int)n, H, nh * D, dt)); rg.rs_n = H; rg.rs_eps = m->rms_eps;
+      SL_TRY(sl_gemm_impl_rows(&a, nullptr, nullptr, &rg, st));
     } else if (sl_family_rows((int)n) > 896 && sl_is16(dt) && L.wgu && rstd_chain && sl_env().decode_tiled) {
       SL_TRY(dec_gemm(m, w, w.att, (int64_t)nh * D, L.wo_dec, x, H, x, (int)n, H, nh * D, SL_ACT_NONE, 0, nullptr, st, nullptr, w.rstd_a, w.h, L.norm2));
       SL_TRY(gemm(dt, w.h, H, L.wgu, H, w.mid, m->ffn, nullptr, nullptr, 0, (int)n, 2 * m->ffn, H, SL_ACT_SILU_MUL, 0, st));
```

New measurement: 67130. 0.974x the previous value.
